# MMAThijssen/catfish

Hardware: NVIDIA B200
Metric: raw_signal_samples_per_sec_resnetrnn_infer (higher is better)
Workload: dtype f16+e5m2 (fp16 product + e5m2 correction product, fp32 accumulate)

## Files before the change

### catfish_b200/build.py

```python

import os
import subprocess
import sys

HERE = os.path.dirname(os.path.abspath(__file__))
CSRC = os.path.join(HERE, "csrc")
INCLUDE = os.path.join(HERE, "..", "include")
LIB = os.environ.get("CF_LIB_OUT") or os.path.join(HERE, "libcatfish_b200.so")
SOURCES = ["api.cu", "k1_normalize.cu", "k6_intervals.cu", "k7_chunks.cu", "k8_split.cu", "k9_validate.cu", "k11_sweep.cu", "simt_engine.cu", "tc_engine.cu"]
NVCC_FLAGS = (["-DCF_PRECISE_ACT"] if os.environ.get("CF_PRECISE_ACT") else []) + os.environ.get("CF_EXTRA_DEFS", "").split() + ["-gencode", "arch=compute_100a,code=sm_100a", "-lineinfo", "-O3", "-std=c++17",
              "--expt-relaxed-constexpr", "-Xcompiler", "-fPIC,-O2,-Wall", "-Xptxas", "-v"]


def _nvcc():
    for cand in (os.environ.get("NVCC"), "/usr/local/cuda/bin/nvcc", "nvcc"):
        if cand and (os.path.sep not in cand or os.path.exists(cand)):
            return cand
    return "nvcc"


def needs_build():
    if not os.path.exists(LIB):
        return True
    t = os.path.getmtime(LIB)
    deps = [os.path.join(CSRC, f) for f in os.listdir(CSRC)] + [os.path.join(INCLUDE, "catfish_b200.h")]
    return any(os.path.getmtime(d) > t for d in deps)


def build(force=False, verbose=False):
    if not force and not needs_build():
        return LIB
    objs = []
    logs = []
    os.makedirs(os.path.join(HERE, "build"), exist_ok=True)
    procs = []
    for src in SOURCES:
        obj = os.path.join(HERE, "build", os.environ.get("CF_OBJ_TAG", "") + src.replace(".cu", ".o"))
        cmd = [_nvcc()] + NVCC_FLAGS + ["-c", os.path.join(CSRC, src), "-o", obj]
        procs.append((src, subprocess.Popen(cmd, stdout=subprocess.PIPE, stderr=subprocess.STDOUT, text=True)))
        objs.append(obj)
    failed = False
    for src, p in procs:
        out, _ = p.communicate()
        logs.append("== %s\n%s" % (src, out))
        if p.returncode != 0:
            failed = True
    log = "\n".join(logs)
    with open(os.path.join(HERE, "build", "nvcc.log"), "w") as f:
        f.write(log)
    if failed:
        sys.stderr.write(log)
        raise RuntimeError("nvcc failed; see catfish_b200/build/nvcc.log")
    cmd = [_nvcc(), "-shared", "-o", LIB] + objs + ["-gencode", "arch=compute_100a,code=sm_100a"]
    r = subprocess.run(cmd, stdout=subprocess.PIPE, stderr=subprocess.STDOUT, text=True)
    if r.returncode != 0:
        sys.stderr.write(r.stdout)
        raise RuntimeError("link failed")
    if verbose:
        print(log)
    return LIB


if __name__ == "__main__":
    print(build(force="--force" in sys.argv, verbose="-v" in sys.argv))
```

### catfish_b200/csrc/tc_engine.cu

```cuda
#include <algorithm>
#include <cmath>
#include <cstdlib>
#include <cstring>
#include <type_traits>

#include "model.cuh"
#include "tc_ptx.cuh"

namespace cf {

using namespace ptx;

constexpr int kH = 64;
constexpr int kC = 32;
constexpr int kNX = 3 * kH;
constexpr int kTcChunkTiles = 2368;
constexpr float kGateScale = -1.4426950408889634f;
constexpr float kCandScale = 2.8853900817779268f;

constexpr int kFmtBf16x3 = 0, kFmtF16E5 = 1;

struct ConvParams {
    static constexpr int kFloats = 10 * 32;
    static constexpr int kW2 = kFloats * 4;
    static constexpr int kW3 = kW2 + 3 * 4096;
    static constexpr int kW45 = kW3 + 4096;
    static constexpr int kW6 = kW45 + 8192;
    static constexpr int kW7 = kW6 + 3 * 4096;
    static constexpr int kBytes = kW7 + 4096;
};

static void pack_b_operand(const float* w, int K, int N, int ldw, int col0, std::vector<__nv_bfloat16>* out,
                           float scale = 1.f, int n_split = 1 << 30, float scale_hi = 1.f) {
    const size_t plane = (size_t)K * N;
    const size_t base = out->size();
    out->resize(base + 2 * plane);
    __nv_bfloat16* hi = out->data() + base;
    __nv_bfloat16* lo = hi + plane;
    for (int k = 0; k < K; ++k)
        for (int n = 0; n < N; ++n) {
            const float v = w[(size_t)k * ldw + col0 + n] * (n < n_split ? scale : scale_hi);
            const __nv_bfloat16 h = __float2bfloat16_rn(v);
            const __nv_bfloat16 l = __float2bfloat16_rn(v - __bfloat162float(h));
            const size_t idx = ((size_t)(k / 8) * N + n) * 8 + (k % 8);
            hi[idx] = h;
            lo[idx] = l;
        }
}

static void pack_b_operand_f16e5(const float* w, int K, int N, int ldw, int col0, std::vector<__nv_bfloat16>* out,
                                 float scale = 1.f, int n_split = 1 << 30, float scale_hi = 1.f) {
    const size_t plane = (size_t)K * N;
    const size_t base = out->size();
    out->resize(base + 2 * plane);
    uint16_t* main = reinterpret_cast<uint16_t*>(out->data() + base);
    uint8_t* corr = reinterpret_cast<uint8_t*>(out->data() + base + plane);
    for (int k = 0; k < K; ++k)
        for (int n = 0; n < N; ++n) {
            const float v = w[(size_t)k * ldw + col0 + n] * (n < n_split ? scale : scale_hi);
            const __half h = __float2half_rn(v);
            const float hf = __half2float(h);
            const __half hs = __float2half_rn(hf * kCorrScale);
            main[((size_t)(k / 8) * N + n) * 8 + (k % 8)] = *reinterpret_cast<const uint16_t*>(&hs);
            const int c = k / 16, kc = k % 16;
            corr[((size_t)(2 * c) * N + n) * 16 + kc] = (uint8_t)__nv_cvt_float_to_fp8(hf / kCorrScale, __NV_SATFINITE, __NV_E5M2);
            corr[((size_t)(2 * c + 1) * N + n) * 16 + kc] = (uint8_t)__nv_cvt_float_to_fp8((v - hf) * kCorrScale, __NV_SATFINITE, __NV_E5M2);
        }
}

struct TcLayer {
    int in = 0;
    DevBuf wfused;
    int fmt = 0;
    DevBuf bz;
    DevBuf wxz;
};

struct TcEngine {
    SimtEnginePtr simt;
    DevBuf conv_params;
    int conv_nres = 0;
    std::vector<TcLayer> layers;
    DevBuf head_w;
    float head_b = 0.f;
    int n_sms = 148;
#ifdef CF_TRACE_PROBES
    bool trace_done = false;
    const char* trace_path = nullptr;
#endif
    int fmt = kFmtBf16x3;
};

bool tc_supported(const HostModel& hm) {
    if (hm.n_res() > 0 && hm.conv_channels() > kC) return false;
    if (hm.n_rnn() > 0 && hm.desc.layer_size > kH) return false;
    return true;
}

static HostModel pad_model(const HostModel& hm) {
    HostModel p = hm;
    if (hm.n_res() > 0) {
        const int C = hm.conv_channels();
        p.desc.layer_size_res = kC;
        for (size_t i = 0; i < hm.convs.size(); ++i) {
            const ConvLayer& s = hm.convs[i];
            ConvLayer& d = p.convs[i];
            const bool scalar_in = i < 2;
            d.cin = scalar_in ? 1 : kC;
            d.cout = kC;
            d.w.assign((size_t)d.k * d.cin * kC, 0.f);
            d.b.assign(kC, 0.f);
            for (int co = 0; co < C; ++co) d.b[co] = s.b[co];
            for (int k = 0; k < s.k; ++k)
                for (int ci = 0; ci < s.cin; ++ci)
                    for (int co = 0; co < C; ++co) d.w[((size_t)k * d.cin + ci) * kC + co] = s.w[((size_t)k * s.cin + ci) * C + co];
        }
    }
    auto unit2 = [](int r, int H) { return r < H ? r : kH + (r - H); };
    if (hm.n_rnn() > 0) {
        const int H = hm.desc.layer_size;
        p.desc.layer_size = kH;
        auto col = [&](int j) { return (j / H) * kH + j % H; };
        for (size_t i = 0; i < hm.gru.size(); ++i) {
            const GruDir& s = hm.gru[i];
            GruDir& d = p.gru[i];
            const bool first = i < 2;
            d.in = first ? (hm.n_res() > 0 ? kC : 1) : 2 * kH;
            d.h = kH;
            d.wx.assign((size_t)d.in * kNX, 0.f);
            d.bx.assign(kNX, 0.f);
            d.wgh.assign((size_t)kH * 2 * kH, 0.f);
            d.wch.assign((size_t)kH * kH, 0.f);
            for (int r = 0; r < s.in; ++r)
                for (int j = 0; j < 3 * H; ++j) d.wx[(size_t)(first ? r : unit2(r, H)) * kNX + col(j)] = s.wx[(size_t)r * 3 * H + j];
            for (int j = 0; j < 3 * H; ++j) d.bx[col(j)] = s.bx[j];
            for (int r = 0; r < H; ++r) {
                for (int j = 0; j < 2 * H; ++j) d.wgh[(size_t)r * 2 * kH + col(j)] = s.wgh[(size_t)r * 2 * H + j];
                for (int j = 0; j < H; ++j) d.wch[(size_t)r * kH + j] = s.wch[(size_t)r * H + j];
            }
        }
        p.head_w.assign(2 * kH, 0.f);
        for (int r = 0; r < 2 * H; ++r) p.head_w[unit2(r, H)] = hm.head_w[r];
    } else {
        p.head_w.assign(kC, 0.f);
        std::copy(hm.head_w.begin(), hm.head_w.end(), p.head_w.begin());
    }
    return p;
}

void EngineDelete::operator()(TcEngine* e) const { delete e; }

static int tc_set_attributes();

int tc_create(const HostModel& narrow, TcEnginePtr* out) {
    CF_TRY(tc_set_attributes());
    TcEnginePtr e(new TcEngine());
    int dev = 0;
    CF_CUDA(cudaGetDevice(&dev));
    CF_CUDA(cudaDeviceGetAttribute(&e->n_sms, cudaDevAttrMultiProcessorCount, dev));
    if (narrow.n_res() == 0) CF_TRY(simt_create(narrow, &e->simt));
    const HostModel hm = pad_model(narrow);
#ifdef CF_TRACE_PROBES
    e->trace_path = getenv("CF_TC_TRACE");
#endif
    {
        const bool covered = (hm.desc.network_type == CF_NET_RESNET_RNN && hm.n_res() == 2 && hm.conv_channels() == kC) ||
                             hm.desc.network_type == CF_NET_RNN;
        float wmax = 0.f;
        for (const GruDir& g : hm.gru) {
            for (float v : g.wx) wmax = std::max(wmax, std::fabs(v));
            for (float v : g.wgh) wmax = std::max(wmax, std::fabs(v));
            for (float v : g.wch) wmax = std::max(wmax, std::fabs(v));
        }
        const bool in_range = wmax * kCandScale * kCorrScale < 60000.f;
        e->fmt = covered && in_range ? kFmtF16E5 : kFmtBf16x3;
    }
    if (hm.n_res() >= 1) {
        const int n_extra = std::max(hm.n_res() - 2, 0);
        std::vector<uint8_t> all((size_t)(1 + n_extra) * ConvParams::kBytes, 0);
        uint8_t* blk = all.data();
        float* fp = reinterpret_cast<float*>(blk);
        auto put = [&](int slot, const std::vector<float>& v) { memcpy(fp + 32 * slot, v.data(), 32 * sizeof(float)); };
        auto put_w = [&](int off, const float* w, int n, int ldw, int col0, int dst_col0, int n_total) {
            __nv_bfloat16* hi = reinterpret_cast<__nv_bfloat16*>(blk + off);
            __nv_bfloat16* lo = hi + 32 * n_total;
            for (int k = 0; k < 32; ++k)
                for (int j = 0; j < n; ++j) {
                    const float v = w[(size_t)k * ldw + col0 + j];
                    const __nv_bfloat16 h = __float2bfloat16_rn(v);
                    const size_t idx = ((size_t)(k / 8) * n_total + dst_col0 + j) * 8 + (k % 8);
                    hi[idx] = h;
                    lo[idx] = __float2bfloat16_rn(v - __bfloat162float(h));
                }
        };
        auto put_block1 = [&](int i) {
            put(6, hm.convs[i].b); put(7, hm.convs[i + 1].b); put(8, hm.convs[i + 2].b); put(9, hm.convs[i + 3].b);
            put_w(ConvParams::kW45, hm.convs[i].w.data(), 32, 32, 0, 0, 64);
            put_w(ConvParams::kW45, hm.convs[i + 1].w.data(), 32, 32, 0, 32, 64);
            for (int tap = 0; tap < 3; ++tap) put_w(ConvParams::kW6 + tap * 4096, hm.convs[i + 2].w.data() + tap * 32 * 32, 32, 32, 0, 0, 32);
            put_w(ConvParams::kW7, hm.convs[i + 3].w.data(), 32, 32, 0, 0, 32);
        };
        put(0, hm.convs[0].w); put(1, hm.convs[0].b);
        put(2, hm.convs[1].w); put(3, hm.convs[1].b);
        put(4, hm.convs[2].b); put(5, hm.convs[3].b);
        for (int tap = 0; tap < 3; ++tap) put_w(ConvParams::kW2 + tap * 4096, hm.convs[2].w.data() + tap * 32 * 32, 32, 32, 0, 0, 32);
        put_w(ConvParams::kW3, hm.convs[3].w.data(), 32, 32, 0, 0, 32);
        if (hm.n_res() >= 2) put_block1(4);
        for (int b = 2; b < hm.n_res(); ++b) {
            blk = all.data() + (size_t)(b - 1) * ConvParams::kBytes;
            fp = reinterpret_cast<float*>(blk);
            put_block1(4 * b);
        }
        CF_TRY(e->conv_params.upload(all));
        e->conv_nres = hm.n_res();
    }
    e->layers.resize(hm.n_rnn());
    for (int l = 0; l < hm.n_rnn(); ++l) {
        TcLayer& L = e->layers[l];
        L.in = hm.gru[2 * l].in;
        L.fmt = L.in == kC ? kFmtBf16x3 : e->fmt;
        std::vector<__nv_bfloat16> wf;
        for (int d = 0; d < 2; ++d) {
            const GruDir& g = hm.gru[2 * l + d];
            auto pack = L.fmt == kFmtF16E5 ? pack_b_operand_f16e5 : pack_b_operand;
            if (L.in > 1) pack(g.wx.data(), L.in, kNX, kNX, 0, &wf, kGateScale, 2 * kH, kCandScale);
            pack(g.wgh.data(), kH, 2 * kH, 2 * kH, 0, &wf, kGateScale, 1 << 30, 1.f);
            pack(g.wch.data(), kH, kH, kH, 0, &wf, kCandScale, 1 << 30, 1.f);
        }
        CF_TRY(L.wfused.upload(wf));
        std::vector<float> bz(2 * kNX);
        for (int d = 0; d < 2; ++d)
            for (int j = 0; j < kNX; ++j)
                bz[d * kNX + j] = hm.gru[2 * l + d].bx[j] * (j < 2 * kH ? kGateScale : kCandScale);
        CF_TRY(L.bz.upload(bz));
        if (L.in == 1) {
            std::vector<float> wxz(2 * kNX);
            for (int d = 0; d < 2; ++d)
                for (int j = 0; j < kNX; ++j)
                    wxz[d * kNX + j] = hm.gru[2 * l + d].wx[j] * (j < 2 * kH ? kGateScale : kCandScale);
            CF_TRY(L.wxz.upload(wxz));
        }
    }
    CF_TRY(e->head_w.upload(hm.head_w));
    e->head_b = hm.head_b;
    *out = std::move(e);
    return CF_OK;
}

int tc_operand_format(const TcEngine* e) { return e ? e->fmt : 0; }
bool tc_can_emit_bits(const TcEngine* e) { return e && !e->layers.empty(); }

constexpr uint32_t kSliceBytes = 2u * 128 * kC * 2;
constexpr uint32_t kConvSmem = ConvParams::kBytes + 10 * kSliceBytes + 35 * 128 * 4 + 256;

__device__ __forceinline__ void store_a_row16(uint8_t* slice, int row, int c0, const float* v) {
#pragma unroll
    for (int g = 0; g < 2; ++g) {
        uint32_t hi[4], lo[4];
#pragma unroll
        for (int i = 0; i < 4; ++i) split_bf16x2(v[g * 8 + 2 * i], v[g * 8 + 2 * i + 1], hi[i], lo[i]);
        uint8_t* dst = slice + (c0 / 8 + g) * 2048 + row * 16;
        *reinterpret_cast<uint4*>(dst) = make_uint4(hi[0], hi[1], hi[2], hi[3]);
        *reinterpret_cast<uint4*>(dst + 8192) = make_uint4(lo[0], lo[1], lo[2], lo[3]);
    }
}

template <int N>
__device__ __forceinline__ void conv_mma_pred(uint32_t tmem_d, uint32_t a_slice, uint32_t w_mat, bool first, uint32_t elected) {
    constexpr uint32_t idesc = make_idesc_bf16(128, N);
#pragma unroll
    for (int pass = 0; pass < 3; ++pass) {
        const uint32_t ap = a_slice + (pass == 1 ? 8192u : 0u);
        const uint32_t wp = w_mat + (pass == 2 ? (uint32_t)(kC * N * 2) : 0u);
#pragma unroll
        for (int kk = 0; kk < 2; ++kk)
            umma_bf16_pred(tmem_d, make_smem_desc(ap + kk * 4096, 2048, 128), make_smem_desc(wp + kk * 2 * (N * 16), N * 16, 128),
                           idesc, !(first && pass == 0 && kk == 0), elected);
    }
}

__global__ void __launch_bounds__(288, 1)
tc_conv2_kernel(const uint8_t* __restrict__ params, const int16_t* __restrict__ raw, const double* __restrict__ stats,
                const float* __restrict__ xwin, const int64_t* __restrict__ src, const int32_t* __restrict__ valid,
                const int32_t* __restrict__ read, int64_t tile0, int n_tiles, __nv_bfloat16* __restrict__ y_out) {
    extern __shared__ __align__(128) uint8_t smem[];
    uint8_t* prm = smem;
    uint8_t* o1 = smem + ConvParams::kBytes;
    uint8_t* o2 = o1 + 4 * kSliceBytes;
    uint8_t* y0 = o2 + kSliceBytes;
    uint8_t* p1 = y0 + kSliceBytes;
    uint8_t* p2 = p1 + 3 * kSliceBytes;
    float* xs = reinterpret_cast<float*>(p2 + kSliceBytes);
    uint64_t* bars = reinterpret_cast<uint64_t*>(xs + 35 * 128);
    uint32_t* tmem_slot = reinterpret_cast<uint32_t*>(bars + 4);
    const float* fp = reinterpret_cast<const float*>(prm);
    uint64_t* bar_ready = &bars[0];
    uint64_t* bar_mma = &bars[1];
    uint64_t* bar_prm = &bars[2];

    const int warp = threadIdx.x >> 5, lane = threadIdx.x & 31;
    if (threadIdx.x == 0) {
        mbar_init(bar_ready, 8);
        mbar_init(bar_mma, 1);
        mbar_init(bar_prm, 1);
        fence_mbar_init();
        mbar_expect_tx(bar_prm, ConvParams::kBytes);
        bulk_g2s(prm, params, ConvParams::kBytes, bar_prm);
    }
    if (warp == 8) tmem_alloc<512>(tmem_slot);
    tc_fence_before_sync();
    __syncthreads();
    tc_fence_after_sync();
    const uint32_t tmem = *tmem_slot;
    constexpr int kLastU = kWindow + 1;
    mbar_wait(bar_prm, 0);

    if (warp == 8) {
        const uint32_t elected = elect_one();
        const uint32_t prm_u = smem_u32(prm);
        const uint32_t o1_u = smem_u32(o1), o2_u = smem_u32(o2);
        uint32_t it = 0;
        for (int tile = blockIdx.x; tile < n_tiles; tile += gridDim.x) {
            for (int u = 0; u <= kLastU; ++u, ++it) {
                mbar_wait(bar_ready, it & 1);
                tc_fence_after_sync();
                const int t1 = u - 1, t2 = u - 2;
                if (t1 >= 0 && t1 < kWindow) {
                    bool first = true;
#pragma unroll
                    for (int tap = 0; tap < 3; ++tap) {
                        const int tt = t1 + tap - 1;
                        if (tt < 0 || tt >= kWindow) continue;
                        conv_mma_pred<32>(tmem + 0, o1_u + (tt & 3) * kSliceBytes, prm_u + ConvParams::kW2 + tap * 4096, first, elected);
                        first = false;
                    }
                }
                if (t2 >= 0 && t2 < kWindow) conv_mma_pred<32>(tmem + 32, o2_u, prm_u + ConvParams::kW3, true, elected);
                umma_commit_pred(bar_mma, elected);
            }
        }
    } else {
        const int q = warp & 3, ch = warp >> 2;
        const int row = q * 32 + lane;
        const int c0 = ch * 16;
        const uint32_t t_lane = tmem + ((uint32_t)(q * 32) << 16) + c0;
        auto relu_bias = [&](uint32_t* r, int slot, float* v) {
#pragma unroll
            for (int i = 0; i < 16; i += 4) {
                const float4 b4 = *reinterpret_cast<const float4*>(fp + 32 * slot + c0 + i);
                v[i] = fmaxf(__uint_as_float(r[i]) + b4.x, 0.f);
                v[i + 1] = fmaxf(__uint_as_float(r[i + 1]) + b4.y, 0.f);
                v[i + 2] = fmaxf(__uint_as_float(r[i + 2]) + b4.z, 0.f);
                v[i + 3] = fmaxf(__uint_as_float(r[i + 3]) + b4.w, 0.f);
            }
        };
        auto make_o1 = [&](int t) {
            const float x = xs[t * 128 + row];
            float v[16];
#pragma unroll
            for (int i = 0; i < 16; ++i) v[i] = fmaxf(fmaf(x, fp[64 + c0 + i], fp[96 + c0 + i]), 0.f);
            store_a_row16(o1 + (t & 3) * kSliceBytes, row, c0, v);
        };
        uint32_t it = 0;
        for (int tile = blockIdx.x; tile < n_tiles; tile += gridDim.x) {
            asm volatile("bar.sync 1, 256;" ::: "memory");
            {
                const int64_t g = (tile0 + tile) * kTileWindows + row;
                const int nv = valid[g];
                const int64_t s0 = src[g];
                double shift = 0.0, scale = 1.0;
                if (raw && nv > 0) { const int r = read[g]; shift = stats[2 * r]; scale = stats[2 * r + 1]; }
                const int tb = ch ? 18 : 0, te = ch ? kWindow : 18;
                for (int t = tb; t < te; ++t) {
                    float v = 0.f;
                    if (t < nv) v = raw ? (float)(((double)raw[s0 + t] - shift) / scale) : xwin[s0 + t];
                    xs[t * 128 + row] = v;
                }
            }
            asm volatile("bar.sync 1, 256;" ::: "memory");
            make_o1(0);
            make_o1(1);
            fence_proxy_async_smem();
            tc_fence_before_sync();
            __syncwarp();
            if (lane == 0) mbar_arrive(bar_ready);
            for (int u = 0; u <= kLastU; ++u, ++it) {
                const int t1 = u - 1, t2 = u - 2;
                const bool h1 = t1 >= 0 && t1 < kWindow, h2 = t2 >= 0 && t2 < kWindow;
                mbar_wait(bar_mma, it & 1);
                tc_fence_after_sync();
                uint32_t r1[16], r2[16];
                if (h1) tmem_ld16_nowait(t_lane + 0, r1);
                if (h2) tmem_ld16_nowait(t_lane + 32, r2);
                tmem_ld_wait();
                tc_fence_before_sync();
                float v[16];
                if (h1) { relu_bias(r1, 4, v); store_a_row16(o2, row, c0, v); }
                if (h2) {
                    relu_bias(r2, 5, v);
                    const float x = xs[t2 * 128 + row];
#pragma unroll
                    for (int i = 0; i < 16; ++i) v[i] = fmaxf(v[i] + fmaf(x, fp[c0 + i], fp[32 + c0 + i]), 0.f);
                    store_a_row16(reinterpret_cast<uint8_t*>(y_out) + ((size_t)tile * kWindow + t2) * kSliceBytes, row, c0, v);
                }
                if (u < kLastU) {
                    fence_proxy_async_smem();
                    __syncwarp();
                    if (lane == 0) mbar_arrive(bar_ready);
                }
                if (u + 2 < kWindow) make_o1(u + 2);
            }
        }
    }
    tc_fence_before_sync();
    __syncthreads();
    if (warp == 8) tmem_dealloc<512>(tmem);
}


template <int FMT>
__device__ __forceinline__ void split4(float v0, float v1, float v2, float v3, int i, uint32_t* m8, uint32_t* s8) {
    if (FMT == kFmtBf16x3) {
        split_bf16x2(v0, v1, m8[i >> 1], s8[i >> 1]);
        split_bf16x2(v2, v3, m8[(i >> 1) + 1], s8[(i >> 1) + 1]);
    } else {
        uint32_t la, lb;
        split_f16e5x2(v0, v1, m8[i >> 1], la);
        split_f16e5x2(v2, v3, m8[(i >> 1) + 1], lb);
        s8[i >> 2] = la | (lb << 16);
        s8[4 + (i >> 2)] = f16e5_hi4(m8[i >> 1], m8[(i >> 1) + 1]);
    }
}

template <int FMT>
__device__ __forceinline__ void store_a_row16_f(uint8_t* slice, int row, int c0, const float* v) {
    uint32_t m8[8], s8[8];
#pragma unroll
    for (int i = 0; i < 16; i += 4) split4<FMT>(v[i], v[i + 1], v[i + 2], v[i + 3], i, m8, s8);
    uint8_t* dst = slice + (c0 / 8) * 2048 + row * 16;
    *reinterpret_cast<uint4*>(dst) = make_uint4(m8[0], m8[1], m8[2], m8[3]);
    *reinterpret_cast<uint4*>(dst + 2048) = make_uint4(m8[4], m8[5], m8[6], m8[7]);
    *reinterpret_cast<uint4*>(dst + 8192) = make_uint4(s8[0], s8[1], s8[2], s8[3]);
    *reinterpret_cast<uint4*>(dst + 8192 + 2048) = make_uint4(s8[4], s8[5], s8[6], s8[7]);
}
template <int FMT>
__device__ __forceinline__ void store_a_tmem16_f(uint32_t t_slot, const float* v) {
    uint32_t m8[8], s8[8];
#pragma unroll
    for (int i = 0; i < 16; i += 4) split4<FMT>(v[i], v[i + 1], v[i + 2], v[i + 3], i, m8, s8);
    tmem_st8_u32(t_slot, m8);
    tmem_st8_u32(t_slot + 16, s8);
}

constexpr uint32_t kConv4Smem = ConvParams::kBytes + 2 * kSliceBytes + 4 * (32 * 128 * 4) + 35 * 128 * 4 + 256;

template <int N>
__device__ __forceinline__ void conv_mma_ts_pred(uint32_t tmem_d, uint32_t tmem_a, uint32_t w_mat, bool first, uint32_t elected) {
    constexpr uint32_t idesc = make_idesc_bf16(128, N);
#pragma unroll
    for (int pass = 0; pass < 3; ++pass) {
        const uint32_t ap = tmem_a + (pass == 1 ? 16u : 0u);
        const uint32_t wp = w_mat + (pass == 2 ? (uint32_t)(kC * N * 2) : 0u);
#pragma unroll
        for (int kk = 0; kk < 2; ++kk)
            umma_bf16_ts_pred(tmem_d, ap + kk * 8, make_smem_desc(wp + kk * 2 * (N * 16), N * 16, 128), idesc,
                              !(first && pass == 0 && kk == 0), elected);
    }
}

__global__ void __launch_bounds__(576, 1)
tc_conv4_kernel(const uint8_t* __restrict__ params, const int16_t* __restrict__ raw, const double* __restrict__ stats,
                const float* __restrict__ xwin, const int64_t* __restrict__ src, const int32_t* __restrict__ valid,
                const int32_t* __restrict__ read, int64_t tile0, int n_tiles, __nv_bfloat16* __restrict__ y_out,
                const float* __restrict__ head_w, float* __restrict__ head_part) {
    constexpr int kFmt = kFmtBf16x3;
    extern __shared__ __align__(128) uint8_t smem[];
    uint8_t* prm = smem;
    uint8_t* o2 = smem + ConvParams::kBytes;
    uint8_t* p2 = o2 + kSliceBytes;
    float* sc_ring = reinterpret_cast<float*>(p2 + kSliceBytes);
    float* xs = sc_ring + 4 * 32 * 128;
    uint64_t* bars = reinterpret_cast<uint64_t*>(xs + 35 * 128);
    uint64_t* bar_ready_x = &bars[0];
    uint64_t* bar_mma_x = &bars[1];
    uint64_t* bar_ready_y = &bars[2];
    uint64_t* bar_mma_y = &bars[3];
    uint64_t* bar_prm = &bars[4];
    uint64_t* bar_y0_full = &bars[5];
    uint64_t* bar_y0_empty = &bars[8];
    uint32_t* tmem_slot = reinterpret_cast<uint32_t*>(bars + 11);
    const float* fp = reinterpret_cast<const float*>(prm);

    const int warp = threadIdx.x >> 5, lane = threadIdx.x & 31;
    if (threadIdx.x == 0) {
        mbar_init(bar_ready_x, 8);
        mbar_init(bar_mma_x, 1);
        mbar_init(bar_ready_y, 8);
        mbar_init(bar_mma_y, 1);
        mbar_init(bar_prm, 1);
        for (int i = 0; i < 3; ++i) { mbar_init(&bar_y0_full[i], 8); mbar_init(&bar_y0_empty[i], 1); }
        fence_mbar_init();
        mbar_expect_tx(bar_prm, ConvParams::kBytes);
        bulk_g2s(prm, params, ConvParams::kBytes, bar_prm);
    }
    if (warp == 16) tmem_alloc<512>(tmem_slot);
    tc_fence_before_sync();
    __syncthreads();
    tc_fence_after_sync();
    const uint32_t tmem = *tmem_slot;
    constexpr int kLastX = kWindow + 1;
    constexpr int kFirstY = 3, kLastY = kWindow + 5;
    constexpr uint32_t kTmScp1 = 128, kTmY0 = 192, kTmO1 = 288, kTmP1 = 416;
    mbar_wait(bar_prm, 0);

    if (warp == 16) {
        const uint32_t elected = elect_one();
        const uint32_t prm_u = smem_u32(prm), o2_u = smem_u32(o2);
        uint32_t it = 0;
        for (int tile = blockIdx.x; tile < n_tiles; tile += gridDim.x) {
            for (int u = 0; u <= kLastX; ++u, ++it) {
                mbar_wait(bar_ready_x, it & 1);
                tc_fence_after_sync();
                const int t1 = u - 1, t2 = u - 2;
                if (t1 >= 0 && t1 < kWindow) {
                    bool first = true;
#pragma unroll
                    for (int tap = 0; tap < 3; ++tap) {
                        const int tt = t1 + tap - 1;
                        if (tt < 0 || tt >= kWindow) continue;
                        conv_mma_ts_pred<32>(tmem + 0, tmem + kTmO1 + (tt & 3) * 32, prm_u + ConvParams::kW2 + tap * 4096, first, elected);
                        first = false;
                    }
                }
                if (t2 >= 0 && t2 < kWindow) conv_mma_pred<32>(tmem + 32, o2_u, prm_u + ConvParams::kW3, true, elected);
                umma_commit_pred(bar_mma_x, elected);
            }
        }
    } else if (warp == 17) {
        const uint32_t elected = elect_one();
        const uint32_t prm_u = smem_u32(prm), p2_u = smem_u32(p2);
        uint32_t it = 0, ny = 0, ny_slot = 0, ny_par = 0;
        for (int tile = blockIdx.x; tile < n_tiles; tile += gridDim.x) {
            for (int u = kFirstY; u <= kLastY; ++u, ++it) {
                mbar_wait(bar_ready_y, it & 1);
                tc_fence_after_sync();
                const int t3 = u - 3, t4 = u - 5, t5 = u - 6;
                if (t3 < kWindow) {
                    mbar_wait(&bar_y0_full[ny_slot], ny_par);
                    tc_fence_after_sync();
                    conv_mma_ts_pred<64>(tmem + kTmScp1, tmem + kTmY0 + ny_slot * 32, prm_u + ConvParams::kW45, true, elected);
                    umma_commit_pred(&bar_y0_empty[ny_slot], elected);
                    ++ny;
                    if (++ny_slot == 3) { ny_slot = 0; ny_par ^= 1; }
                }
                if (t4 >= 0 && t4 < kWindow) {
                    bool first = true;
#pragma unroll
                    for (int tap = 0; tap < 3; ++tap) {
                        const int tt = t4 + tap - 1;
                        if (tt < 0 || tt >= kWindow) continue;
                        conv_mma_ts_pred<32>(tmem + 64, tmem + kTmP1 + (tt % 3) * 32, prm_u + ConvParams::kW6 + tap * 4096, first, elected);
                        first = false;
                    }
                }
                if (t5 >= 0 && t5 < kWindow) conv_mma_pred<32>(tmem + 96, p2_u, prm_u + ConvParams::kW7, true, elected);
                umma_commit_pred(bar_mma_y, elected);
            }
        }
    } else {
        const int ew = warp & 7;
        const int q = ew & 3, ch = ew >> 2;
        const int row = q * 32 + lane;
        const int c0 = ch * 16;
        const uint32_t t_row = tmem + ((uint32_t)(q * 32) << 16);
        const uint32_t t_lane = t_row + c0;
        const uint32_t t_opnd = t_row + ch * 8;
        auto relu_bias = [&](uint32_t* r, int slot, float* v) {
#pragma unroll
            for (int i = 0; i < 16; i += 4) {
                const float4 b4 = *reinterpret_cast<const float4*>(fp + 32 * slot + c0 + i);
                const float2 s0 = fadd2(make_float2(__uint_as_float(r[i]), __uint_as_float(r[i + 1])), make_float2(b4.x, b4.y));
                const float2 s1 = fadd2(make_float2(__uint_as_float(r[i + 2]), __uint_as_float(r[i + 3])), make_float2(b4.z, b4.w));
                v[i] = fmaxf(s0.x, 0.f);
                v[i + 1] = fmaxf(s0.y, 0.f);
                v[i + 2] = fmaxf(s1.x, 0.f);
                v[i + 3] = fmaxf(s1.y, 0.f);
            }
        };
        if (warp < 8) {
            auto make_o1 = [&](int t) {
                const float2 x = splat2(xs[t * 128 + row]);
                float v[16];
#pragma unroll
                for (int i = 0; i < 16; i += 2) {
                    const float2 o = ffma2(x, *reinterpret_cast<const float2*>(fp + 64 + c0 + i), *reinterpret_cast<const float2*>(fp + 96 + c0 + i));
                    v[i] = fmaxf(o.x, 0.f);
                    v[i + 1] = fmaxf(o.y, 0.f);
                }
                store_a_tmem16_f<kFmt>(t_opnd + kTmO1 + (t & 3) * 32, v);
            };
            uint32_t it = 0, ny = 0, ny_slot = 0, ny_par = 1;
            for (int tile = blockIdx.x; tile < n_tiles; tile += gridDim.x) {
                asm volatile("bar.sync 1, 256;" ::: "memory");
                {
                    const int64_t g = (tile0 + tile) * kTileWindows + row;
                    const int nv = valid[g];
                    const int64_t s0 = src[g];
                    double shift = 0.0, scale = 1.0;
                    if (raw && nv > 0) { const int r = read[g]; shift = stats[2 * r]; scale = stats[2 * r + 1]; }
                    const int tb = ch ? 18 : 0, te = ch ? kWindow : 18;
                    for (int t = tb; t < te; ++t) {
                        float v = 0.f;
                        if (t < nv) v = raw ? (float)(((double)raw[s0 + t] - shift) / scale) : xwin[s0 + t];
                        xs[t * 128 + row] = v;
                    }
                }
                asm volatile("bar.sync 1, 256;" ::: "memory");
                make_o1(0);
                make_o1(1);
                tmem_st_wait();
                tc_fence_before_sync();
                __syncwarp();
                if (lane == 0) mbar_arrive(bar_ready_x);
                for (int u = 0; u <= kLastX; ++u, ++it) {
                    const int t1 = u - 1, t2 = u - 2;
                    const bool h1 = t1 >= 0 && t1 < kWindow, h2 = t2 >= 0 && t2 < kWindow;
                    mbar_wait(bar_mma_x, it & 1);
                    tc_fence_after_sync();
                    uint32_t r1[16], r2[16];
                    if (h1) tmem_ld16_nowait(t_lane + 0, r1);
                    if (h2) tmem_ld16_nowait(t_lane + 32, r2);
                    tmem_ld_wait();
                    float v[16];
                    if (h1) { relu_bias(r1, 4, v); store_a_row16_f<kFmt>(o2, row, c0, v); }
                    if (u < kLastX) {
                        fence_proxy_async_smem();
                        tmem_st_wait();
                        tc_fence_before_sync();
                        __syncwarp();
                        if (lane == 0) mbar_arrive(bar_ready_x);
                    }
                    if (h2) {
                        relu_bias(r2, 5, v);
                        const float2 x = splat2(xs[t2 * 128 + row]);
#pragma unroll
                        for (int i = 0; i < 16; i += 2) {
                            const float2 sc = ffma2(x, *reinterpret_cast<const float2*>(fp + c0 + i), *reinterpret_cast<const float2*>(fp + 32 + c0 + i));
                            const float2 o = fadd2(make_float2(v[i], v[i + 1]), sc);
                            v[i] = fmaxf(o.x, 0.f);
                            v[i + 1] = fmaxf(o.y, 0.f);
                        }
                        if (ny >= 3) mbar_wait(&bar_y0_empty[ny_slot], ny_par);
                        tc_fence_after_sync();
                        store_a_tmem16_f<kFmt>(t_opnd + kTmY0 + ny_slot * 32, v);
                        tmem_st_wait();
                        tc_fence_before_sync();
                        __syncwarp();
                        if (lane == 0) mbar_arrive(&bar_y0_full[ny_slot]);
                        ++ny;
                        if (++ny_slot == 3) { ny_slot = 0; ny_par ^= 1; }
                    }
                    if (u + 2 < kWindow) make_o1(u + 2);
                }
            }
        } else {
            float* sc_mine = sc_ring + c0 * 128 + row;
            uint32_t it = 0;
            if (lane == 0) mbar_arrive(bar_ready_y);
            for (int tile = blockIdx.x; tile < n_tiles; tile += gridDim.x) {
                for (int u = kFirstY; u <= kLastY; ++u, ++it) {
                    const int t3 = u - 3, t4 = u - 5, t5 = u - 6;
                    const bool h3 = t3 < kWindow, h4 = t4 >= 0 && t4 < kWindow, h5 = t5 >= 0 && t5 < kWindow;
                    mbar_wait(bar_mma_y, it & 1);
                    tc_fence_after_sync();
                    uint32_t r3[16], r4[16], r5[16], rs[16];
                    if (h3) {
                        tmem_ld16_nowait(t_lane + kTmScp1 + 32, r3);
                        tmem_ld16_nowait(t_lane + kTmScp1, rs);
                    }
                    if (h4) tmem_ld16_nowait(t_lane + 64, r4);
                    if (h5) tmem_ld16_nowait(t_lane + 96, r5);
                    tmem_ld_wait();
                    float v[16];
                    if (h3) { relu_bias(r3, 7, v); store_a_tmem16_f<kFmt>(t_opnd + kTmP1 + (t3 % 3) * 32, v); }
                    if (h4) { relu_bias(r4, 8, v); store_a_row16_f<kFmt>(p2, row, c0, v); }
                    fence_proxy_async_smem();
                    tmem_st_wait();
                    tc_fence_before_sync();
                    __syncwarp();
                    if (lane == 0) mbar_arrive(bar_ready_y);
                    if (h3) {
                        float* dst = sc_mine + (t3 & 3) * 4096;
#pragma unroll
                        for (int i = 0; i < 16; ++i) dst[i * 128] = __uint_as_float(rs[i]) + fp[192 + c0 + i];
                    }
                    if (h5) {
                        relu_bias(r5, 9, v);
                        const float* sc = sc_mine + (t5 & 3) * 4096;
#pragma unroll
                        for (int i = 0; i < 16; i += 2) {
                            const float2 o = fadd2(make_float2(v[i], v[i + 1]), make_float2(sc[i * 128], sc[(i + 1) * 128]));
                            v[i] = fmaxf(o.x, 0.f);
                            v[i + 1] = fmaxf(o.y, 0.f);
                        }
                        if (head_w) {
                            float2 acc2 = make_float2(0.f, 0.f);
#pragma unroll
                            for (int i = 0; i < 16; i += 2)
                                acc2 = ffma2(make_float2(v[i], v[i + 1]), __ldg(reinterpret_cast<const float2*>(head_w + c0 + i)), acc2);
                            head_part[(((size_t)tile * kWindow + t5) * 2 + ch) * 128 + row] = acc2.x + acc2.y;
                        } else {
                            store_a_row16_f<kFmt>(reinterpret_cast<uint8_t*>(y_out) + ((size_t)tile * kWindow + t5) * kSliceBytes, row, c0, v);
                        }
                    }
                }
            }
        }
    }
    tc_fence_before_sync();
    __syncthreads();
    if (warp == 16) tmem_dealloc<512>(tmem);
}

constexpr int kBlockRing = 4;
constexpr uint32_t kBlockSmem = ConvParams::kBytes + (kBlockRing + 3 + 1) * kSliceBytes + 256;

__global__ void __launch_bounds__(320, 1)
tc_conv_block_kernel(const uint8_t* __restrict__ params, const __nv_bfloat16* __restrict__ y_in, int n_tiles,
                     __nv_bfloat16* __restrict__ y_out) {
    constexpr int kFmt = kFmtBf16x3;
    extern __shared__ __align__(128) uint8_t smem[];
    uint8_t* prm = smem;
    uint8_t* yin = smem + ConvParams::kBytes;
    uint8_t* p1 = yin + kBlockRing * kSliceBytes;
    uint8_t* p2 = p1 + 3 * kSliceBytes;
    uint64_t* bars = reinterpret_cast<uint64_t*>(p2 + kSliceBytes);
    uint64_t* bar_ready = &bars[0];
    uint64_t* bar_mma = &bars[1];
    uint64_t* bar_prm = &bars[2];
    uint64_t* bar_full = &bars[3];
    uint64_t* bar_empty = &bars[3 + kBlockRing];
    uint32_t* tmem_slot = reinterpret_cast<uint32_t*>(bars + 3 + 2 * kBlockRing);
    const float* fp = reinterpret_cast<const float*>(prm);

    const int warp = threadIdx.x >> 5, lane = threadIdx.x & 31;
    if (threadIdx.x == 0) {
        mbar_init(bar_ready, 8);
        mbar_init(bar_mma, 1);
        mbar_init(bar_prm, 1);
        for (int i = 0; i < kBlockRing; ++i) { mbar_init(&bar_full[i], 1); mbar_init(&bar_empty[i], 1); }
        fence_mbar_init();
        mbar_expect_tx(bar_prm, ConvParams::kBytes);
        bulk_g2s(prm, params, ConvParams::kBytes, bar_prm);
    }
    if (warp == 8) tmem_alloc<512>(tmem_slot);
    tc_fence_before_sync();
    __syncthreads();
    tc_fence_after_sync();
    const uint32_t tmem = *tmem_slot;
    constexpr int kLastU = kWindow + 2;
    constexpr uint32_t kTmP2 = 256, kTmP3 = 288;
    mbar_wait(bar_prm, 0);

    if (warp == 8) {
        const uint32_t elected = elect_one();
        const uint32_t prm_u = smem_u32(prm), yin_u = smem_u32(yin), p1_u = smem_u32(p1), p2_u = smem_u32(p2);
        uint32_t it = 0, n = 0;
        for (int tile = blockIdx.x; tile < n_tiles; tile += gridDim.x) {
            for (int u = 0; u <= kLastU; ++u, ++it) {
                mbar_wait(bar_ready, it & 1);
                tc_fence_after_sync();
                const int t2 = u - 2, t3 = u - 3;
                if (u < kWindow) {
                    const uint32_t slot = n % kBlockRing;
                    mbar_wait(&bar_full[slot], (n / kBlockRing) & 1);
                    conv_mma_pred<64>(tmem + (u & 3) * 64, yin_u + slot * kSliceBytes, prm_u + ConvParams::kW45, true, elected);
                    umma_commit_pred(&bar_empty[slot], elected);
                    ++n;
                }
                if (t2 >= 0 && t2 < kWindow) {
                    bool first = true;
#pragma unroll
                    for (int tap = 0; tap < 3; ++tap) {
                        const int tt = t2 + tap - 1;
                        if (tt < 0 || tt >= kWindow) continue;
                        conv_mma_pred<32>(tmem + kTmP2, p1_u + (tt % 3) * kSliceBytes, prm_u + ConvParams::kW6 + tap * 4096, first, elected);
                        first = false;
                    }
                }
                if (t3 >= 0 && t3 < kWindow) conv_mma_pred<32>(tmem + kTmP3, p2_u, prm_u + ConvParams::kW7, true, elected);
                umma_commit_pred(bar_mma, elected);
            }
        }
    } else if (warp == 9) {
        if (lane == 0) {
            const uint8_t* src = reinterpret_cast<const uint8_t*>(y_in);
            uint32_t n = 0;
            for (int tile = blockIdx.x; tile < n_tiles; tile += gridDim.x)
                for (int t = 0; t < kWindow; ++t, ++n) {
                    const uint32_t slot = n % kBlockRing;
                    if (n >= kBlockRing) mbar_wait(&bar_empty[slot], (n / kBlockRing - 1) & 1);
                    mbar_expect_tx(&bar_full[slot], kSliceBytes);
                    bulk_g2s(yin + slot * kSliceBytes, src + ((size_t)tile * kWindow + t) * kSliceBytes, kSliceBytes, &bar_full[slot]);
                }
        }
    } else {
        const int q = warp & 3, ch = warp >> 2;
        const int row = q * 32 + lane;
        const int c0 = ch * 16;
        const uint32_t t_lane = tmem + ((uint32_t)(q * 32) << 16) + c0;
        auto relu_bias = [&](uint32_t* r, int slot, float* v) {
#pragma unroll
            for (int i = 0; i < 16; i += 4) {
                const float4 b4 = *reinterpret_cast<const float4*>(fp + 32 * slot + c0 + i);
                const float2 s0 = fadd2(make_float2(__uint_as_float(r[i]), __uint_as_float(r[i + 1])), make_float2(b4.x, b4.y));
                const float2 s1 = fadd2(make_float2(__uint_as_float(r[i + 2]), __uint_as_float(r[i + 3])), make_float2(b4.z, b4.w));
                v[i] = fmaxf(s0.x, 0.f);
                v[i + 1] = fmaxf(s0.y, 0.f);
                v[i + 2] = fmaxf(s1.x, 0.f);
                v[i + 3] = fmaxf(s1.y, 0.f);
            }
        };
        uint32_t it = 0;
        if (lane == 0) mbar_arrive(bar_ready);
        for (int tile = blockIdx.x; tile < n_tiles; tile += gridDim.x) {
            for (int u = 0; u <= kLastU; ++u, ++it) {
                const int t2 = u - 2, t3 = u - 3;
                const bool h1 = u < kWindow, h2 = t2 >= 0 && t2 < kWindow, h3 = t3 >= 0 && t3 < kWindow;
                mbar_wait(bar_mma, it & 1);
                tc_fence_after_sync();
                uint32_t r1[16], r2[16], r3[16], rs[16];
                if (h1) tmem_ld16_nowait(t_lane + (u & 3) * 64 + 32, r1);
                if (h2) tmem_ld16_nowait(t_lane + kTmP2, r2);
                if (h3) {
                    tmem_ld16_nowait(t_lane + kTmP3, r3);
                    tmem_ld16_nowait(t_lane + (t3 & 3) * 64, rs);
                }
                tmem_ld_wait();
                float v[16];
                if (h1) { relu_bias(r1, 7, v); store_a_row16_f<kFmt>(p1 + (u % 3) * kSliceBytes, row, c0, v); }
                if (h2) { relu_bias(r2, 8, v); store_a_row16_f<kFmt>(p2, row, c0, v); }
                fence_proxy_async_smem();
                tc_fence_before_sync();
                __syncwarp();
                if (lane == 0) mbar_arrive(bar_ready);
                if (h3) {
                    relu_bias(r3, 9, v);
#pragma unroll
                    for (int i = 0; i < 16; i += 2) {
                        const float2 sc = fadd2(make_float2(__uint_as_float(rs[i]), __uint_as_float(rs[i + 1])),
                                                *reinterpret_cast<const float2*>(fp + 192 + c0 + i));
                        const float2 o = fadd2(make_float2(v[i], v[i + 1]), sc);
                        v[i] = fmaxf(o.x, 0.f);
                        v[i + 1] = fmaxf(o.y, 0.f);
                    }
                    store_a_row16_f<kFmt>(reinterpret_cast<uint8_t*>(y_out) + ((size_t)tile * kWindow + t3) * kSliceBytes, row, c0, v);
                }
            }
        }
    }
    tc_fence_before_sync();
    __syncthreads();
    if (warp == 8) tmem_dealloc<512>(tmem);
}

template <int KX> struct GruF2Cfg {
    static constexpr bool kNoX = KX == 1;
    static constexpr int kChunks = KX / 16;
    static constexpr int kStages = KX == 128 ? 8 : 10;
    static constexpr uint32_t kWx = 0;
    static constexpr uint32_t kWgh = kWx + (kNoX ? 0u : 2u * KX * kNX * 2);
    static constexpr uint32_t kWch = kWgh + 2u * kH * 128 * 2;
    static constexpr uint32_t kWBytes = kWch + 2u * kH * 64 * 2;
    static constexpr uint32_t kRing = kWBytes;
    static constexpr uint32_t kBias = kRing + (uint32_t)kStages * 8192;
    static constexpr uint32_t kBars = kBias + 2 * 192 * 4;
    static constexpr uint32_t kSmem = kBars + 512;
    static constexpr int kBarG = 0, kBarC = 1, kBarRh = 2, kBarH = 3, kBarCfree = 4, kBarXdone = 5;
    static constexpr int kBarFull = 16, kBarEmpty = 16 + kStages, kBarTma = 16 + 2 * kStages, kBarW = 16 + 3 * kStages;
};
__host__ __device__ constexpr uint32_t gru_out_block_bytes(int fmt) { return fmt == kFmtF16E5 ? 49152u : 65536u; }
constexpr int kGruF2Threads = 768;
constexpr int kGruF2Converters = 2;
constexpr int kGruF2EpiRegs = 96, kGruF2ServiceRegs = 48;

template <int KX, int FMT, int FMT_OUT>
__global__ void __launch_bounds__(kGruF2Threads, 1)
tc_gru_fused2_kernel(const uint8_t* __restrict__ wpk, const float* __restrict__ bias,
                     const __nv_bfloat16* __restrict__ x_blocks, __nv_bfloat16* __restrict__ y_out,
                     const float* __restrict__ head_w, float* __restrict__ head_part, int n_tiles,
                     long long* __restrict__ trace, const float* __restrict__ x_scalar, const float* __restrict__ wx_scalar) {
    using Cfg = GruF2Cfg<KX>;
    constexpr bool kNoX = Cfg::kNoX;
#ifdef CF_TRACE_PROBES
    int tr_n = 0;
#define CF_TR(region, step, tag)                                                                   \
    do {                                                                                           \
        if (trace && blockIdx.x == 0 && (step) >= 36 && (step) < 40 && tr_n < 200) {               \
            trace[((region) * 200 + tr_n) * 2] = (tag) + 1000 * (long long)(step);                      \
            trace[((region) * 200 + tr_n) * 2 + 1] = clock64();                                    \
            ++tr_n;                                                                                \
        }                                                                                          \
    } while (0)
#else
#define CF_TR(region, step, tag) do { } while (0)
#endif
#ifdef CF_TRACE_CHUNKS
#define CF_TRC(region, step, tag) CF_TR(region, step, tag)
#else
#define CF_TRC(region, step, tag) do { } while (0)
#endif
    extern __shared__ __align__(128) uint8_t smem[];
    uint64_t* bars = reinterpret_cast<uint64_t*>(smem + Cfg::kBars);
    uint64_t* w_bar = &bars[Cfg::kBarW];
    uint32_t* tmem_slot = reinterpret_cast<uint32_t*>(&bars[Cfg::kBarW + 1]);
    float* bias_s = reinterpret_cast<float*>(smem + Cfg::kBias);

    const int warp = threadIdx.x >> 5, lane = threadIdx.x & 31;
    const int dir = blockIdx.x & 1;
    const int slot = blockIdx.x >> 1, n_slots = gridDim.x >> 1;
    const int stride = 2 * n_slots;
    auto tiles_of = [&](int chain) -> int {
        const int first = slot * 2 + chain;
        return first < n_tiles ? (n_tiles - first + stride - 1) / stride : 0;
    };
    auto blk_of = [&](int chain, int gs) -> size_t {
        const int ti = gs / kWindow, s = gs - ti * kWindow;
        return (size_t)(slot * 2 + chain + ti * stride) * kWindow + (dir ? kWindow - 1 - s : s);
    };

    if (threadIdx.x == 0) {
        for (int c = 0; c < 2; ++c) {
            uint64_t* b = &bars[8 * c];
            mbar_init(&b[Cfg::kBarG], 1);
            mbar_init(&b[Cfg::kBarC], 1);
            mbar_init(&b[Cfg::kBarRh], 16);
            mbar_init(&b[Cfg::kBarH], 16);
            mbar_init(&b[Cfg::kBarCfree], 16);
            mbar_init(&b[Cfg::kBarXdone], 1);
        }
        for (int i = 0; i < Cfg::kStages; ++i) {
            mbar_init(&bars[Cfg::kBarFull + i], 1);
            mbar_init(&bars[Cfg::kBarEmpty + i], 1);
            mbar_init(&bars[Cfg::kBarTma + i], 1);
        }
        mbar_init(w_bar, 1);
        fence_mbar_init();
    }
#ifndef CF_PRECISE_ACT
    if (threadIdx.x < 192) bias_s[threadIdx.x] = bias[dir * kNX + threadIdx.x] * (threadIdx.x < 2 * kH ? kSigArgScale : kTanhArgScale);
    if (kNoX && threadIdx.x < 192) bias_s[192 + threadIdx.x] = wx_scalar[dir * kNX + threadIdx.x] * (threadIdx.x < 2 * kH ? kSigArgScale : kTanhArgScale);
#else
    if (threadIdx.x < 192) bias_s[threadIdx.x] = bias[dir * kNX + threadIdx.x];
    if (kNoX && threadIdx.x < 192) bias_s[192 + threadIdx.x] = wx_scalar[dir * kNX + threadIdx.x];
#endif
    if (warp == 16) tmem_alloc<512>(tmem_slot);
    tc_fence_before_sync();
    __syncthreads();
    tc_fence_after_sync();
    const uint32_t tmem = *tmem_slot;

    if (warp >= 16) {
    asm volatile("setmaxnreg.dec.sync.aligned.u32 %0;" ::"n"(kGruF2ServiceRegs));
    if (warp == 18) {
        if (lane == 0) {
            mbar_expect_tx(w_bar, Cfg::kWBytes);
            const uint8_t* wsrc = wpk + (size_t)dir * Cfg::kWBytes;
            for (uint32_t off = 0; off < Cfg::kWBytes; off += 32768) {
                const uint32_t n = Cfg::kWBytes - off < 32768 ? Cfg::kWBytes - off : 32768;
                bulk_g2s(smem + off, wsrc + off, n, w_bar);
            }
            constexpr bool kCompact = FMT == kFmtF16E5;
            constexpr size_t plane = (size_t)128 * KX * 2;
            constexpr size_t blk_bytes = kCompact ? plane + (size_t)(KX / 16) * 2048 : 2 * plane;
            const uint8_t* xbase = reinterpret_cast<const uint8_t*>(x_blocks);
            const int total0 = tiles_of(0) * kWindow, total1 = tiles_of(1) * kWindow;
            uint32_t st = 0, par = 1;
            for (int gs = 0; gs < (kNoX ? 0 : total0); ++gs) {
                for (int c = 0; c < 2; ++c) {
                    if (c == 1 && gs >= total1) break;
                    const uint8_t* xb = xbase + blk_of(c, gs) * blk_bytes;
                    if (kCompact) {
                        const int nc = (c == 0 && gs < total1) ? 1 : 0, ngs = nc ? gs : gs + 1;
                        if (ngs < total0 && (nc == 0 || ngs < total1)) {
                            const uint8_t* nb = xbase + blk_of(nc, ngs) * blk_bytes;
                            bulk_prefetch_l2(nb, (uint32_t)plane);
                            bulk_prefetch_l2(nb + plane, (uint32_t)(KX / 16) * 2048);
                        }
                    }
                    for (int kk = 0; kk < Cfg::kChunks; ++kk) {
                        mbar_wait(&bars[Cfg::kBarEmpty + st], par);
                        CF_TRC(5, gs, 80 + kk);
                        uint8_t* dst = smem + Cfg::kRing + st * 8192;
                        uint64_t* landed = &bars[(kCompact ? Cfg::kBarTma : Cfg::kBarFull) + st];
                        if (kCompact) {
                            mbar_expect_tx(landed, 6144);
                            bulk_g2s(dst, xb + kk * 4096, 4096, landed);
                            bulk_g2s(dst + 4096, xb + plane + kk * 2048, 2048, landed);
                        } else {
                            mbar_expect_tx(landed, 8192);
                            bulk_g2s(dst, xb + kk * 4096, 4096, landed);
                            bulk_g2s(dst + 4096, xb + plane + kk * 4096, 4096, landed);
                        }
                        if (++st == Cfg::kStages) { st = 0; par ^= 1; }
                    }
                }
            }
        }
    } else if (warp >= 19) {
        if (FMT == kFmtF16E5 && warp < 19 + kGruF2Converters) {
            static_assert(Cfg::kStages % kGruF2Converters == 0, "converter warps split the ring by stage");
            const int total0 = tiles_of(0) * kWindow, total1 = tiles_of(1) * kWindow;
            const int n_chunks = (total0 + total1) * Cfg::kChunks;
            uint32_t st = warp - 19, par = 0;
            for (int cn = warp - 19; cn < n_chunks; cn += kGruF2Converters) {
                mbar_wait(&bars[Cfg::kBarTma + st], par);
                if (lane == 0 && warp == 19) CF_TRC(4, cn / (2 * Cfg::kChunks), 70);
                uint8_t* stage = smem + Cfg::kRing + st * 8192;
#pragma unroll
                for (int r = 0; r < 4; ++r) {
                    const int row = r * 32 + lane;
                    const uint4 a = *reinterpret_cast<const uint4*>(stage + row * 16);
                    const uint4 b = *reinterpret_cast<const uint4*>(stage + 2048 + row * 16);
                    *reinterpret_cast<uint4*>(stage + 6144 + row * 16) =
                        make_uint4(f16e5_hi4(a.x, a.y), f16e5_hi4(a.z, a.w), f16e5_hi4(b.x, b.y), f16e5_hi4(b.z, b.w));
                }
                fence_proxy_async_smem();
                __syncwarp();
                if (lane == 0) mbar_arrive(&bars[Cfg::kBarFull + st]);
                if (lane == 0 && warp == 19) CF_TRC(4, cn / (2 * Cfg::kChunks), 71);
                if ((st += kGruF2Converters) >= Cfg::kStages) { st -= Cfg::kStages; par ^= 1; }
            }
        }
    } else if (warp >= 16 && warp < 18) {
        {
            constexpr bool kE5 = FMT == kFmtF16E5;
            constexpr uint32_t idesc_g = kE5 ? make_idesc_f16(128, 2 * kH) : make_idesc_bf16(128, 2 * kH);
            constexpr uint32_t idesc_c = kE5 ? make_idesc_f16(128, kH) : make_idesc_bf16(128, kH);
            constexpr uint32_t idesc_x = kE5 ? make_idesc_f16(128, kNX) : make_idesc_bf16(128, kNX);
            constexpr uint32_t idesc_g8 = make_idesc_e5m2(128, 2 * kH), idesc_c8 = make_idesc_e5m2(128, kH);
            constexpr uint32_t idesc_x8 = make_idesc_e5m2(128, kNX);
            const uint32_t elected = elect_one();
            const int c = warp - 16;
            const uint32_t s0 = smem_u32(smem);
            uint64_t* b = &bars[8 * c];
            const uint32_t dg = tmem + c * 256, dc = dg + 2 * kH, ta = dg + 3 * kH;
            const int total = tiles_of(c) * kWindow;
            const int total1 = tiles_of(1) * kWindow;
            mbar_wait(w_bar, 0);
            for (int gs = 0; gs < total; ++gs) {
                const uint32_t par = gs & 1;
                uint32_t cn = (uint32_t)(c == 0 ? gs + (gs < total1 ? gs : total1) : 2 * gs + 1) * Cfg::kChunks;
                if (kNoX) {
                } else if (c == 1) mbar_wait(&bars[Cfg::kBarXdone], gs & 1);
                else if (gs > 0 && gs - 1 < total1) mbar_wait(&bars[8 + Cfg::kBarXdone], (gs - 1) & 1);
                if (gs > 0) mbar_wait(&b[Cfg::kBarCfree], (gs - 1) & 1);
                if (lane == 0) CF_TR(c, gs, 10);
                auto issue_x = [&](auto st0c) {
                    constexpr int kSt0 = decltype(st0c)::value;
                    static_assert(kSt0 + Cfg::kChunks <= Cfg::kStages || kNoX, "an entry does not wrap around the ring");
                    uint32_t ring_lo = (uint32_t)make_smem_desc(s0 + Cfg::kRing, 2048, 128);
                    uint32_t wx_lo = (uint32_t)make_smem_desc(s0 + Cfg::kWx, kNX * 16, 128);
                    asm volatile("" : "+r"(ring_lo), "+r"(wx_lo));
                    constexpr uint64_t ahi = make_smem_desc(0, 2048, 128) & 0xffffffff00000000ull;
                    constexpr uint64_t bhi = make_smem_desc(0, kNX * 16, 128) & 0xffffffff00000000ull;
                    const uint32_t xpar = (cn / Cfg::kStages) & 1;
#pragma unroll
                    for (int kk = 0; kk < Cfg::kChunks; ++kk) {
                        const int st = kSt0 + kk;
                        mbar_wait(&bars[Cfg::kBarFull + st], xpar);
                        if (lane == 0) CF_TRC(c, gs, 60 + kk);
                        tc_fence_after_sync();
                        const uint32_t a_lo = ring_lo + st * (8192 >> 4), w_lo = wx_lo + kk * (2 * kNX * 16 >> 4);
                        if (kE5) {
                            umma_bf16_pred(dg, ahi | a_lo, bhi | w_lo, idesc_x, kk != 0, elected);
                            umma_f8_pred(dg, ahi | (a_lo + (4096 >> 4)), bhi | (w_lo + (KX * kNX * 2 >> 4)), idesc_x8, 1, elected);
                        } else {
#pragma unroll
                            for (int pass = 0; pass < 3; ++pass)
                                umma_bf16_pred(dg, ahi | (a_lo + (pass == 1 ? 4096 >> 4 : 0)),
                                               bhi | (w_lo + (pass == 2 ? KX * kNX * 2 >> 4 : 0)), idesc_x, (kk | pass) != 0, elected);
                        }
                        umma_commit_pred(&bars[Cfg::kBarEmpty + st], elected);
                        if (lane == 0) CF_TRC(c, gs, 20 + kk);
                        if (kk == Cfg::kChunks - 1 && lane == 0) CF_TR(c, gs, 27);
                    }
                };
                if constexpr (kNoX) {
                } else if constexpr (Cfg::kChunks == Cfg::kStages) {
                    issue_x(std::integral_constant<int, 0>{});
                } else {
                    static_assert(Cfg::kStages == 10 && Cfg::kChunks == 2, "entries start at the even stages 0..8");
                    switch (cn % Cfg::kStages) {
                        case 0: issue_x(std::integral_constant<int, 0>{}); break;
                        case 2: issue_x(std::integral_constant<int, 2>{}); break;
                        case 4: issue_x(std::integral_constant<int, 4>{}); break;
                        case 6: issue_x(std::integral_constant<int, 6>{}); break;
                        default: issue_x(std::integral_constant<int, 8>{}); break;
                    }
                }
                if (!kNoX && lane == 0) mbar_arrive(&b[Cfg::kBarXdone]);
                uint32_t wgh_lo = (uint32_t)make_smem_desc(s0 + Cfg::kWgh, 128 * 16, 128);
                uint32_t wch_lo = (uint32_t)make_smem_desc(s0 + Cfg::kWch, 64 * 16, 128);
                asm volatile("" : "+r"(wgh_lo), "+r"(wch_lo));
                constexpr uint64_t ghi = make_smem_desc(0, 128 * 16, 128) & 0xffffffff00000000ull;
                constexpr uint64_t chi = make_smem_desc(0, 64 * 16, 128) & 0xffffffff00000000ull;
                mbar_wait(&b[Cfg::kBarH], par);
                if (lane == 0) CF_TR(c, gs, 30);
                tc_fence_after_sync();
                if (kE5) {
#pragma unroll
                    for (int kk = 0; kk < kH / 16; ++kk) {
                        const uint32_t w_lo = wgh_lo + kk * (2 * 128 * 16 >> 4);
                        umma_bf16_ts_pred(dg, ta + kk * 8, ghi | w_lo, idesc_g, !kNoX || kk != 0, elected);
                        umma_f8_ts_pred(dg, ta + 32 + kk * 8, ghi | (w_lo + (kH * 128 * 2 >> 4)), idesc_g8, 1, elected);
                    }
                } else {
#pragma unroll
                    for (int pass = 0; pass < 3; ++pass) {
                        const uint32_t ap = ta + (pass == 1 ? 32u : 0u);
#pragma unroll
                        for (int kk = 0; kk < kH / 16; ++kk)
                            umma_bf16_ts_pred(dg, ap + kk * 8, ghi | (wgh_lo + (pass == 2 ? kH * 128 * 2 >> 4 : 0) + kk * (2 * 128 * 16 >> 4)),
                                              idesc_g, !kNoX || (pass | kk) != 0, elected);
                    }
                }
                umma_commit_pred(&b[Cfg::kBarG], elected);
                if (lane == 0) CF_TR(c, gs, 31);
                mbar_wait(&b[Cfg::kBarRh], par);
                if (lane == 0) CF_TR(c, gs, 40);
                tc_fence_after_sync();
                if (kE5) {
#pragma unroll
                    for (int kk = 0; kk < kH / 16; ++kk) {
                        const uint32_t w_lo = wch_lo + kk * (2 * 64 * 16 >> 4);
                        umma_bf16_ts_pred(dc, ta + kk * 8, chi | w_lo, idesc_c, !kNoX || kk != 0, elected);
                        umma_f8_ts_pred(dc, ta + 32 + kk * 8, chi | (w_lo + (kH * 64 * 2 >> 4)), idesc_c8, 1, elected);
                    }
                } else {
#pragma unroll
                    for (int pass = 0; pass < 3; ++pass) {
                        const uint32_t ap = ta + (pass == 1 ? 32u : 0u);
#pragma unroll
                        for (int kk = 0; kk < kH / 16; ++kk)
                            umma_bf16_ts_pred(dc, ap + kk * 8, chi | (wch_lo + (pass == 2 ? kH * 64 * 2 >> 4 : 0) + kk * (2 * 64 * 16 >> 4)),
                                              idesc_c, !kNoX || (pass | kk) != 0, elected);
                    }
                }
                umma_commit_pred(&b[Cfg::kBarC], elected);
                if (lane == 0) CF_TR(c, gs, 41);
            }
        }
    }
    } else {
        asm volatile("setmaxnreg.inc.sync.aligned.u32 %0;" ::"n"(kGruF2EpiRegs));
        const int q = warp & 3, us = warp >> 2;
        const int row = q * 32 + lane;
        const int j0 = us * 16;
        const uint32_t t_row = tmem + ((uint32_t)(q * 32) << 16);
        const int tot[2] = {tiles_of(0) * kWindow, tiles_of(1) * kWindow};
        float2 h2[2][8];
        int spos[2] = {0, 0};
        const uint32_t blk_step = dir ? 0xffffffffu : 1u;
        const uint32_t blk_jump = (uint32_t)stride * kWindow - blk_step * (kWindow - 1);
        uint32_t cblk[2] = {(uint32_t)(slot * 2) * kWindow + (dir ? kWindow - 1 : 0),
                            (uint32_t)(slot * 2 + 1) * kWindow + (dir ? kWindow - 1 : 0)};
        uint8_t* const y_main = reinterpret_cast<uint8_t*>(y_out) + ((size_t)(dir * kH + j0) / 8 * 128 + row) * 16;
        const int32_t y_lo_delta = FMT_OUT == kFmtF16E5
            ? 128 * 2 * kH * 2 + ((dir * kH + j0) / 16 * 128 + row) * 16 - ((dir * kH + j0) / 8 * 128 + row) * 16
            : 128 * 2 * kH * 2;
        float* const head_base = head_part + (dir * 4 + us) * 128 + row;
        const float* const xs_base = x_scalar + row;
#pragma unroll
        for (int c = 0; c < 2; ++c)
#pragma unroll
            for (int j = 0; j < 8; ++j) h2[c][j] = make_float2(0.f, 0.f);

        auto bias4 = [&](int idx, float xv) -> float4 {
            float4 b4 = *reinterpret_cast<const float4*>(bias_s + idx);
            if (kNoX) {
                const float4 w4 = *reinterpret_cast<const float4*>(bias_s + 192 + idx);
                b4.x = fmaf(xv, w4.x, b4.x); b4.y = fmaf(xv, w4.y, b4.y); b4.z = fmaf(xv, w4.z, b4.z); b4.w = fmaf(xv, w4.w, b4.w);
            }
            return b4;
        };
        auto sig4 = [&](const uint32_t* a, float4 b4, float2& o0, float2& o1) {
#ifndef CF_PRECISE_ACT
            o0 = sigmoid_zb2(make_float2(__uint_as_float(a[0]), __uint_as_float(a[1])), make_float2(b4.x, b4.y));
            o1 = sigmoid_zb2(make_float2(__uint_as_float(a[2]), __uint_as_float(a[3])), make_float2(b4.z, b4.w));
#else
            float z[4] = {__uint_as_float(a[0]) + b4.x, __uint_as_float(a[1]) + b4.y, __uint_as_float(a[2]) + b4.z, __uint_as_float(a[3]) + b4.w};
            float y[4];
            sigmoid4_z(z, y);
            o0 = make_float2(y[0], y[1]);
            o1 = make_float2(y[2], y[3]);
#endif
        };
        auto tanh4v = [&](const uint32_t* a, float4 b4, float2& o0, float2& o1) {
#ifndef CF_PRECISE_ACT
            o0 = tanh_zb2(make_float2(__uint_as_float(a[0]), __uint_as_float(a[1])), make_float2(b4.x, b4.y));
            o1 = tanh_zb2(make_float2(__uint_as_float(a[2]), __uint_as_float(a[3])), make_float2(b4.z, b4.w));
#else
            float z[4] = {__uint_as_float(a[0]) + b4.x, __uint_as_float(a[1]) + b4.y, __uint_as_float(a[2]) + b4.z, __uint_as_float(a[3]) + b4.w};
            float y[4];
            tanh4_z(z, y);
            o0 = make_float2(y[0], y[1]);
            o1 = make_float2(y[2], y[3]);
#endif
        };
        auto begin_tile = [&](int c) {
            const uint32_t t_ahi = t_row + c * 256 + 3 * kH + j0 / 2, t_alo = t_ahi + 32;
            const uint32_t z[8] = {0, 0, 0, 0, 0, 0, 0, 0};
#pragma unroll
            for (int j = 0; j < 8; ++j) h2[c][j] = make_float2(0.f, 0.f);
            tmem_st8_u32(t_ahi, z);
            tmem_st8_u32(t_alo, z);
            tmem_st_wait();
            tc_fence_before_sync();
            __syncwarp();
            if (lane == 0) mbar_arrive(&bars[8 * c + Cfg::kBarH]);
        };
        auto phase_r = [&](int c, int gs) {
            uint64_t* b = &bars[8 * c];
            const uint32_t t_acc = t_row + c * 256 + j0;
            const uint32_t t_ahi = t_row + c * 256 + 3 * kH + j0 / 2, t_alo = t_ahi + 32;
            const float xv = kNoX ? __ldg(xs_base + (size_t)cblk[c] * 128) : 0.f;
            if (warp == 0 && lane == 0) CF_TR(2 + c, gs, 49);
            mbar_wait(&b[Cfg::kBarG], gs & 1);
            if (warp == 0 && lane == 0) CF_TR(2 + c, gs, 50);
            tc_fence_after_sync();
            uint32_t ar[16];
            tmem_ld16_nowait(t_acc, ar);
            tmem_ld_wait();
            uint32_t hi[8], lo[8];
#pragma unroll
            for (int i = 0; i < 16; i += 4) {
                float2 r0, r1;
                sig4(ar + i, bias4(j0 + i, xv), r0, r1);
                const float2 p0 = fmul2(r0, h2[c][i >> 1]), p1 = fmul2(r1, h2[c][(i >> 1) + 1]);
                split4<FMT>(p0.x, p0.y, p1.x, p1.y, i, hi, lo);
            }
            tmem_st8_u32(t_ahi, hi);
            tmem_st8_u32(t_alo, lo);
            tmem_st_wait();
            tc_fence_before_sync();
            __syncwarp();
            if (lane == 0) mbar_arrive(&b[Cfg::kBarRh]);
            if (warp == 0 && lane == 0) CF_TR(2 + c, gs, 51);
        };
        auto phase_c = [&](int c, int gs) {
            uint64_t* b = &bars[8 * c];
            const uint32_t t_acc = t_row + c * 256 + j0;
            const uint32_t t_ahi = t_row + c * 256 + 3 * kH + j0 / 2, t_alo = t_ahi + 32;
            const uint32_t blk = cblk[c];
            const int s = spos[c];
            const float xv = kNoX ? __ldg(xs_base + (size_t)blk * 128) : 0.f;
            float2 u2[8];
            {
                uint32_t au[16];
                tmem_ld16_nowait(t_acc + kH, au);
                tmem_ld_wait();
#pragma unroll
                for (int i = 0; i < 16; i += 4) sig4(au + i, bias4(kH + j0 + i, xv), u2[i >> 1], u2[(i >> 1) + 1]);
            }
            if (warp == 0 && lane == 0) CF_TR(2 + c, gs, 52);
            mbar_wait(&b[Cfg::kBarC], gs & 1);
            if (warp == 0 && lane == 0) CF_TR(2 + c, gs, 53);
            tc_fence_after_sync();
            uint32_t ac[16];
            tmem_ld16_nowait(t_acc + 2 * kH, ac);
            tmem_ld_wait();
            tc_fence_before_sync();
            __syncwarp();
            if (lane == 0) mbar_arrive(&b[Cfg::kBarCfree]);
            uint32_t hi[8], lo[8];
#pragma unroll
            for (int i = 0; i < 16; i += 4) {
                float2 c0v, c1v;
                tanh4v(ac + i, bias4(2 * kH + j0 + i, xv), c0v, c1v);
                float2& ha = h2[c][i >> 1];
                float2& hb = h2[c][(i >> 1) + 1];
                ha = ffma2(u2[i >> 1], ffma2(c0v, splat2(-1.f), ha), c0v);
                hb = ffma2(u2[(i >> 1) + 1], ffma2(c1v, splat2(-1.f), hb), c1v);
                split4<FMT>(ha.x, ha.y, hb.x, hb.y, i, hi, lo);
            }
            const bool more = gs + 1 < tot[c];
            if (s + 1 < kWindow) {
                tmem_st8_u32(t_ahi, hi);
                tmem_st8_u32(t_alo, lo);
                tmem_st_wait();
                tc_fence_before_sync();
                __syncwarp();
                if (lane == 0) mbar_arrive(&b[Cfg::kBarH]);
            }
            if (warp == 0 && lane == 0) CF_TR(2 + c, gs, 55);
            if (y_out) {
                if (FMT_OUT != FMT) {
#pragma unroll
                    for (int i = 0; i < 16; i += 4)
                        split4<FMT_OUT>(h2[c][i >> 1].x, h2[c][i >> 1].y, h2[c][(i >> 1) + 1].x, h2[c][(i >> 1) + 1].y, i, hi, lo);
                }
                uint8_t* ym = y_main + (size_t)blk * gru_out_block_bytes(FMT_OUT);
                *reinterpret_cast<uint4*>(ym) = make_uint4(hi[0], hi[1], hi[2], hi[3]);
                *reinterpret_cast<uint4*>(ym + 2048) = make_uint4(hi[4], hi[5], hi[6], hi[7]);
                *reinterpret_cast<uint4*>(ym + y_lo_delta) = make_uint4(lo[0], lo[1], lo[2], lo[3]);
                if (FMT_OUT != kFmtF16E5)
                    *reinterpret_cast<uint4*>(ym + y_lo_delta + 2048) = make_uint4(lo[4], lo[5], lo[6], lo[7]);
            }
            if (head_part) {
                const float* hw = head_w + dir * kH + j0;
                float2 acc2 = make_float2(0.f, 0.f);
#pragma unroll
                for (int i = 0; i < 8; ++i) acc2 = ffma2(h2[c][i], __ldg(reinterpret_cast<const float2*>(hw) + i), acc2);
                head_base[(size_t)blk * 1024] = acc2.x + acc2.y;
            }
            if (s + 1 == kWindow) {
                spos[c] = 0;
                cblk[c] = blk + blk_jump;
                if (more) begin_tile(c);
            } else {
                spos[c] = s + 1;
                cblk[c] = blk + blk_step;
            }
            if (warp == 0 && lane == 0) CF_TR(2 + c, gs, 56);
        };

        if (tot[0] > 0) begin_tile(0);
        if (tot[1] > 0) begin_tile(1);
        const int g_end = tot[0] > tot[1] ? tot[0] : tot[1];
        for (int g = 0; g <= g_end; ++g) {
            if (g < tot[0]) phase_r(0, g);
            if (g >= 1 && g - 1 < tot[1]) phase_c(1, g - 1);
            if (g < tot[0]) phase_c(0, g);
            if (g < tot[1]) phase_r(1, g);
        }
    }
    tc_fence_before_sync();
    __syncthreads();
    if (warp == 16) tmem_dealloc<512>(tmem);
}

#undef CF_TR
#undef CF_TRC

__global__ void __launch_bounds__(256)
tc_head_kernel(const float* __restrict__ head_part, int n_parts, float b, const int64_t* __restrict__ src,
               const int32_t* __restrict__ valid, const int32_t* __restrict__ read,
               const double* __restrict__ stats, int64_t tile0, int64_t n_rows, float* __restrict__ probs, int want_logits,
               unsigned* __restrict__ lwords, double threshold) {
    __shared__ float logit[kWindow][kTileWindows + 1];
    const int64_t tile = blockIdx.x;
    if (tile * kTileWindows * kWindow >= n_rows) return;
    for (int i = threadIdx.x; i < kWindow * kTileWindows; i += blockDim.x) {
        const int t = i / kTileWindows, w = i % kTileWindows;
        const size_t blk = (size_t)tile * kWindow + t;
        float acc = b;
        for (int k = 0; k < n_parts; ++k) acc += head_part[(blk * n_parts + k) * 128 + w];
        logit[t][w] = acc;
    }
    __syncthreads();
    for (int i = threadIdx.x; i < kWindow * kTileWindows; i += blockDim.x) {
        const int w = i / kWindow, t = i % kWindow;
        const int64_t g = (tile0 + tile) * kTileWindows + w;
        const bool real = t < valid[g];
        float p = 0.f;
        if (real) {
            p = want_logits ? logit[t][w] : 1.f / (1.f + expf(-logit[t][w]));
            if (stats) {
                const double sc = stats[2 * read[g] + 1];
                if (!(sc > 0.0)) p = nanf("");
            }
        }
        if (!lwords) {
            if (real) probs[src[g] + t] = p;
            continue;
        }
        const bool hit = real && (double)p >= threshold;
        const unsigned hits = __ballot_sync(0xffffffffu, hit);
        if (hit) {
            const int64_t sidx = src[g] + t;
            const unsigned peers = __match_any_sync(hits, (unsigned long long)(sidx >> 5));
            const unsigned bits = __reduce_or_sync(peers, 1u << (sidx & 31));
            if ((threadIdx.x & 31) == __ffs(peers) - 1) atomicOr(&lwords[sidx >> 5], bits);
        }
    }
}

__global__ void __launch_bounds__(256)
tc_head_conv_kernel(const __nv_bfloat16* __restrict__ y, const float* __restrict__ w, float b,
                    const int64_t* __restrict__ src, const int32_t* __restrict__ valid,
                    const int32_t* __restrict__ read, const double* __restrict__ stats,
                    int64_t tile0, int64_t n_rows, float* __restrict__ probs, int want_logits) {
    __shared__ float logit[kWindow][kTileWindows + 1];
    __shared__ float ws[kC];
    const int64_t tile = blockIdx.x;
    if (tile * kTileWindows * kWindow >= n_rows) return;
    if (threadIdx.x < kC) ws[threadIdx.x] = w[threadIdx.x];
    __syncthreads();
    for (int i = threadIdx.x; i < kWindow * kTileWindows; i += blockDim.x) {
        const int t = i / kTileWindows, wr = i % kTileWindows;
        const __nv_bfloat16* blk = y + ((size_t)tile * kWindow + t) * (2 * 128 * kC);
        float acc = b;
#pragma unroll
        for (int kg = 0; kg < kC / 8; ++kg) {
            const uint4 hi = *reinterpret_cast<const uint4*>(blk + ((size_t)kg * 128 + wr) * 8);
            const uint4 lo = *reinterpret_cast<const uint4*>(blk + 128 * kC + ((size_t)kg * 128 + wr) * 8);
            const uint32_t hw[4] = {hi.x, hi.y, hi.z, hi.w}, lw[4] = {lo.x, lo.y, lo.z, lo.w};
#pragma unroll
            for (int k = 0; k < 4; ++k) {
                const float v0 = __uint_as_float(hw[k] << 16) + __uint_as_float(lw[k] << 16);
                const float v1 = __uint_as_float(hw[k] & 0xffff0000u) + __uint_as_float(lw[k] & 0xffff0000u);
                acc = fmaf(v0, ws[kg * 8 + 2 * k], acc);
                acc = fmaf(v1, ws[kg * 8 + 2 * k + 1], acc);
            }
        }
        logit[t][wr] = acc;
    }
    __syncthreads();
    for (int i = threadIdx.x; i < kWindow * kTileWindows; i += blockDim.x) {
        const int wr = i / kWindow, t = i % kWindow;
        const int64_t g = (tile0 + tile) * kTileWindows + wr;
        if (t >= valid[g]) continue;
        float p = want_logits ? logit[t][wr] : 1.f / (1.f + expf(-logit[t][wr]));
        if (stats) {
            const double sc = stats[2 * read[g] + 1];
            if (!(sc > 0.0)) p = nanf("");
        }
        probs[src[g] + t] = p;
    }
}

int simt_conv_stack(SimtEngine* e, DevBuf* ws, const HostModel& hm, const int16_t* raw, const double* stats,
                    const float* xwin, WindowTable tab, int64_t tile0, int64_t tiles, int64_t chunk_tiles,
                    const float** feat, cudaStream_t stream, Profiler* prof);

static size_t tc_workspace_bytes(int64_t tiles) {
    const size_t blocks = (size_t)tiles * kWindow;
    size_t b = 0;
    b += blocks * 128 * kC * 2 * 2;
    b += 2 * blocks * 128 * 2 * kH * 2 * 2;
    b += blocks * 8 * 128 * 4;
    return b + 4096;
}

int tc_reserve(const TcEngine* e, DevBuf* ws, DevBuf* simt_ws, const HostModel& hm, int64_t n_tiles) {
    if (n_tiles <= 0) return CF_OK;
    const int64_t chunk = n_tiles < kTcChunkTiles ? n_tiles : kTcChunkTiles;
    CF_TRY(ws->ensure(tc_workspace_bytes(chunk)));
    if (!e->conv_params.ptr) CF_TRY(simt_conv_stack_reserve(simt_ws, hm, chunk));
    return CF_OK;
}

constexpr uint32_t kSmemPerSm = 228 * 1024;
static_assert(GruF2Cfg<128>::kSmem > kSmemPerSm / 2, "two tc_gru_fused2_kernel<128> CTAs could share an SM's TMEM");
static_assert(GruF2Cfg<32>::kSmem > kSmemPerSm / 2, "two tc_gru_fused2_kernel<32> CTAs could share an SM's TMEM");
static_assert(GruF2Cfg<1>::kSmem > kSmemPerSm / 2, "two tc_gru_fused2_kernel<1> CTAs could share an SM's TMEM");
static_assert(kConv4Smem > kSmemPerSm / 2, "two tc_conv4_kernel CTAs could share an SM's TMEM");
static_assert(kBlockSmem > kSmemPerSm / 2, "two tc_conv_block_kernel CTAs could share an SM's TMEM");
static_assert(kConvSmem > kSmemPerSm / 2, "two tc_conv2_kernel CTAs could share an SM's TMEM");

static int tc_set_attributes() {
    CF_CUDA(cudaFuncSetAttribute(tc_gru_fused2_kernel<1, 0, 0>, cudaFuncAttributeMaxDynamicSharedMemorySize, GruF2Cfg<1>::kSmem));
    CF_CUDA(cudaFuncSetAttribute(tc_gru_fused2_kernel<1, 1, 1>, cudaFuncAttributeMaxDynamicSharedMemorySize, GruF2Cfg<1>::kSmem));
    CF_CUDA(cudaFuncSetAttribute(tc_gru_fused2_kernel<32, 0, 0>, cudaFuncAttributeMaxDynamicSharedMemorySize, GruF2Cfg<32>::kSmem));
    CF_CUDA(cudaFuncSetAttribute(tc_gru_fused2_kernel<32, 0, 1>, cudaFuncAttributeMaxDynamicSharedMemorySize, GruF2Cfg<32>::kSmem));
    CF_CUDA(cudaFuncSetAttribute(tc_gru_fused2_kernel<128, 0, 0>, cudaFuncAttributeMaxDynamicSharedMemorySize, GruF2Cfg<128>::kSmem));
    CF_CUDA(cudaFuncSetAttribute(tc_gru_fused2_kernel<128, 1, 1>, cudaFuncAttributeMaxDynamicSharedMemorySize, GruF2Cfg<128>::kSmem));
    CF_CUDA(cudaFuncSetAttribute(tc_conv2_kernel, cudaFuncAttributeMaxDynamicSharedMemorySize, kConvSmem));
    CF_CUDA(cudaFuncSetAttribute(tc_conv4_kernel, cudaFuncAttributeMaxDynamicSharedMemorySize, kConv4Smem));
    CF_CUDA(cudaFuncSetAttribute(tc_conv_block_kernel, cudaFuncAttributeMaxDynamicSharedMemorySize, kBlockSmem));
    return CF_OK;
}

int tc_forward(TcEngine* e, DevBuf* ws, DevBuf* simt_ws, const HostModel& hm, const int16_t* raw, const double* stats,
               const float* xwin, WindowTable tab, int64_t n_tiles, float* probs, cudaStream_t stream, Profiler* prof,
               bool want_logits, const LabelBits* bits) {
    if (n_tiles <= 0) return CF_OK;
    if (bits && (e->layers.empty() || want_logits)) { set_error("label-bit output needs a GRU head"); return CF_ERR_BAD_ARG; }
    const int64_t chunk = n_tiles < kTcChunkTiles ? n_tiles : kTcChunkTiles;
    CF_TRY(ws->ensure(tc_workspace_bytes(chunk)));
    const size_t blocks_max = (size_t)chunk * kWindow;
    uint8_t* p = static_cast<uint8_t*>(ws->ptr);
    __nv_bfloat16* a0 = reinterpret_cast<__nv_bfloat16*>(p);
    p += blocks_max * 128 * kC * 2 * 2;
    __nv_bfloat16* ybuf[2];
    ybuf[0] = reinterpret_cast<__nv_bfloat16*>(p);
    p += blocks_max * 128 * 2 * kH * 2 * 2;
    ybuf[1] = reinterpret_cast<__nv_bfloat16*>(p);
    p += blocks_max * 128 * 2 * kH * 2 * 2;
    float* head_part = reinterpret_cast<float*>(p);

    const int n_layers = (int)e->layers.size();
    for (int64_t tile0 = 0; tile0 < n_tiles; tile0 += kTcChunkTiles) {
        const int64_t tiles = std::min<int64_t>(kTcChunkTiles, n_tiles - tile0);
        const int64_t blocks = tiles * kWindow;
        const int64_t rows = blocks * 128;
        const float* feat = nullptr;
        const __nv_bfloat16* a_in = nullptr;
        if (e->conv_params.ptr) {
            ProfScope ps(prof, KC_K2_CONV, stream);
            const int grid = (int)std::min<int64_t>(tiles, e->n_sms);
            const bool fused_head = n_layers == 0 && e->conv_nres == 2;
            if (e->conv_nres >= 2)
                tc_conv4_kernel<<<grid, 576, kConv4Smem, stream>>>(e->conv_params.as<uint8_t>(), raw, stats, xwin, tab.src,
                                                                  tab.valid, tab.read, tile0, (int)tiles, a0,
                                                                  fused_head ? e->head_w.as<float>() : nullptr,
                                                                  fused_head ? head_part : nullptr);
            else
                tc_conv2_kernel<<<grid, 288, kConvSmem, stream>>>(e->conv_params.as<uint8_t>(), raw, stats, xwin, tab.src, tab.valid,
                                                                  tab.read, tile0, (int)tiles, a0);
            CF_LAUNCHED();
            a_in = a0;
            for (int b = 2; b < e->conv_nres; ++b) {
                __nv_bfloat16* out = a_in == a0 ? ybuf[1] : a0;
                tc_conv_block_kernel<<<grid, 320, kBlockSmem, stream>>>(
                    e->conv_params.as<uint8_t>() + (size_t)(b - 1) * ConvParams::kBytes, a_in, (int)tiles, out);
                CF_LAUNCHED();
                a_in = out;
            }
        } else {
            CF_TRY(simt_conv_stack(e->simt.get(), simt_ws, hm, raw, stats, xwin, tab, tile0, tiles, chunk, &feat, stream, prof));
        }
        for (int l = 0; l < n_layers; ++l) {
            const TcLayer& L = e->layers[l];
            const bool last = l + 1 == n_layers;
            __nv_bfloat16* yo = last ? nullptr : ybuf[l & 1];
            ProfScope ps(prof, KC_K4_GRU, stream);
            long long* trace_dev = nullptr;
#ifdef CF_TRACE_PROBES
            if (e->trace_path && !e->trace_done && L.in != kC) {
                CF_CUDA(cudaMalloc(&trace_dev, 6 * 200 * 2 * sizeof(long long)));
                CF_CUDA(cudaMemsetAsync(trace_dev, 0, 6 * 200 * 2 * sizeof(long long), stream));
            }
#endif
            const int grid2 = 2 * (int)std::min<int64_t>((tiles + 1) / 2, e->n_sms / 2);
            const float* hw_l = last ? e->head_w.as<float>() : nullptr;
            float* hp_l = last ? head_part : nullptr;
            const int fmt_out = last ? L.fmt : e->layers[l + 1].fmt;
            if (L.in == 1) {
                if (L.fmt == kFmtF16E5)
                    tc_gru_fused2_kernel<1, 1, 1><<<grid2, kGruF2Threads, GruF2Cfg<1>::kSmem, stream>>>(
                        L.wfused.as<uint8_t>(), L.bz.as<float>(), nullptr, yo, hw_l, hp_l, (int)tiles, nullptr, feat, L.wxz.as<float>());
                else
                    tc_gru_fused2_kernel<1, 0, 0><<<grid2, kGruF2Threads, GruF2Cfg<1>::kSmem, stream>>>(
                        L.wfused.as<uint8_t>(), L.bz.as<float>(), nullptr, yo, hw_l, hp_l, (int)tiles, nullptr, feat, L.wxz.as<float>());
            } else if (L.in == kC) {
                if (fmt_out == kFmtF16E5)
                    tc_gru_fused2_kernel<32, 0, 1><<<grid2, kGruF2Threads, GruF2Cfg<32>::kSmem, stream>>>(
                        L.wfused.as<uint8_t>(), L.bz.as<float>(), a_in, yo, hw_l, hp_l, (int)tiles, nullptr, nullptr, nullptr);
                else
                    tc_gru_fused2_kernel<32, 0, 0><<<grid2, kGruF2Threads, GruF2Cfg<32>::kSmem, stream>>>(
                        L.wfused.as<uint8_t>(), L.bz.as<float>(), a_in, yo, hw_l, hp_l, (int)tiles, nullptr, nullptr, nullptr);
            } else if (L.fmt == kFmtF16E5) {
                tc_gru_fused2_kernel<128, 1, 1><<<grid2, kGruF2Threads, GruF2Cfg<128>::kSmem, stream>>>(
                    L.wfused.as<uint8_t>(), L.bz.as<float>(), a_in, yo, hw_l, hp_l, (int)tiles, trace_dev, nullptr, nullptr);
            } else {
                tc_gru_fused2_kernel<128, 0, 0><<<grid2, kGruF2Threads, GruF2Cfg<128>::kSmem, stream>>>(
                    L.wfused.as<uint8_t>(), L.bz.as<float>(), a_in, yo, hw_l, hp_l, (int)tiles, trace_dev, nullptr, nullptr);
            }
            CF_LAUNCHED();
#ifdef CF_TRACE_PROBES
            if (trace_dev) {
                CF_CUDA(cudaStreamSynchronize(stream));
                std::vector<long long> host(6 * 200 * 2);
                CF_CUDA(cudaMemcpy(host.data(), trace_dev, host.size() * sizeof(long long), cudaMemcpyDeviceToHost));
                if (FILE* f = fopen(e->trace_path, "w")) {
                    for (int rg = 0; rg < 6; ++rg)
                        for (int k = 0; k < 200; ++k)
                            if (host[(rg * 200 + k) * 2 + 1])
                                fprintf(f, "%d %lld %lld\n", rg, host[(rg * 200 + k) * 2], host[(rg * 200 + k) * 2 + 1]);
                    fclose(f);
                }
                cudaFree(trace_dev);
                e->trace_done = true;
            }
#endif
            a_in = yo;
        }
        if (n_layers == 0 && e->conv_nres == 2) {
            ProfScope ps(prof, KC_K5_HEAD, stream);
            tc_head_kernel<<<(unsigned)tiles, 256, 0, stream>>>(
                head_part, 2, e->head_b, tab.src, tab.valid, tab.read, raw ? stats : nullptr, tile0, rows, probs, want_logits ? 1 : 0,
                nullptr, 0.0);
            CF_LAUNCHED();
        } else if (n_layers == 0) {
            ProfScope ps(prof, KC_K5_HEAD, stream);
            tc_head_conv_kernel<<<(unsigned)tiles, 256, 0, stream>>>(
                a_in, e->head_w.as<float>(), e->head_b, tab.src, tab.valid, tab.read, raw ? stats : nullptr, tile0, rows, probs, want_logits ? 1 : 0);
            CF_LAUNCHED();
        } else {
            ProfScope ps(prof, KC_K5_HEAD, stream);
            tc_head_kernel<<<(unsigned)tiles, 256, 0, stream>>>(
                head_part, 8, e->head_b, tab.src, tab.valid, tab.read, raw ? stats : nullptr, tile0, rows, probs, want_logits ? 1 : 0,
                bits ? bits->lwords : nullptr, bits ? bits->threshold : 0.0);
            CF_LAUNCHED();
        }
    }
    return CF_OK;
}

__global__ void __launch_bounds__(128, 1)
tc_selftest_f16e5_kernel(const float* __restrict__ a, const uint8_t* __restrict__ wpk, int K, int N, int mode,
                         float* __restrict__ out) {
    extern __shared__ __align__(128) uint8_t smem[];
    uint8_t* a_s = smem;
    uint8_t* w_s = smem + 128 * K * 4;
    uint64_t* bar = reinterpret_cast<uint64_t*>(w_s + (size_t)N * K * 4);
    uint32_t* tmem_slot = reinterpret_cast<uint32_t*>(bar + 1);
    const int row = threadIdx.x, warp = threadIdx.x >> 5;
    if (threadIdx.x == 0) { mbar_init(bar, 1); fence_mbar_init(); }
    if (warp == 0) tmem_alloc<256>(tmem_slot);
    for (int i = threadIdx.x; i < N * K * 4 / 16; i += 128)
        reinterpret_cast<uint4*>(w_s)[i] = reinterpret_cast<const uint4*>(wpk)[i];
    tc_fence_before_sync();
    __syncthreads();
    tc_fence_after_sync();
    const uint32_t tmem = *tmem_slot;
    const uint32_t t_row = tmem + ((uint32_t)(warp * 32) << 16);
    constexpr uint32_t kTmA = 128;
    for (int c = 0; c < K / 16; ++c) {
        float v[16];
        for (int i = 0; i < 16; ++i) v[i] = a[(size_t)row * K + 16 * c + i];
        uint32_t m8[8], lo4[4], hi4[4];
        split_f16e5_chunk(v, m8, lo4, hi4);
        if (mode == 0) {
            *reinterpret_cast<uint4*>(a_s + (2 * c) * 2048 + row * 16) = make_uint4(m8[0], m8[1], m8[2], m8[3]);
            *reinterpret_cast<uint4*>(a_s + (2 * c + 1) * 2048 + row * 16) = make_uint4(m8[4], m8[5], m8[6], m8[7]);
            uint8_t* corr = a_s + 128 * K * 2;
            *reinterpret_cast<uint4*>(corr + (2 * c) * 2048 + row * 16) = make_uint4(lo4[0], lo4[1], lo4[2], lo4[3]);
            *reinterpret_cast<uint4*>(corr + (2 * c + 1) * 2048 + row * 16) = make_uint4(hi4[0], hi4[1], hi4[2], hi4[3]);
        } else {
            uint32_t c8[8] = {lo4[0], lo4[1], lo4[2], lo4[3], hi4[0], hi4[1], hi4[2], hi4[3]};
            tmem_st8_u32(t_row + kTmA + 16 * c, m8);
            tmem_st8_u32(t_row + kTmA + 16 * c + 8, c8);
        }
    }
    fence_proxy_async_smem();
    tmem_st_wait();
    tc_fence_before_sync();
    __syncthreads();
    if (warp == 0) {
        tc_fence_after_sync();
        const uint32_t elected = elect_one();
        const uint32_t a_u = smem_u32(a_s), w_u = smem_u32(w_s);
        const uint32_t id16 = make_idesc_f16(128, N), id8 = make_idesc_e5m2(128, N);
        for (int c = 0; c < K / 16; ++c) {
            const uint64_t bm = make_smem_desc(w_u + c * 2 * (N * 16), N * 16, 128);
            const uint64_t bc = make_smem_desc(w_u + K * N * 2 + c * 2 * (N * 16), N * 16, 128);
            if (mode == 0) {
                umma_bf16_pred(tmem, make_smem_desc(a_u + c * 4096, 2048, 128), bm, id16, c > 0, elected);
                umma_f8_pred(tmem, make_smem_desc(a_u + 128 * K * 2 + c * 4096, 2048, 128), bc, id8, 1, elected);
            } else {
                umma_bf16_ts_pred(tmem, tmem + kTmA + 16 * c, bm, id16, c > 0, elected);
                umma_f8_ts_pred(tmem, tmem + kTmA + 16 * c + 8, bc, id8, 1, elected);
            }
        }
        umma_commit_pred(bar, elected);
    }
    mbar_wait(bar, 0);
    tc_fence_after_sync();
    for (int n0 = 0; n0 < N; n0 += 16) {
        float v[16];
        tmem_ld16(t_row + n0, v);
        for (int i = 0; i < 16; ++i) out[(size_t)row * N + n0 + i] = v[i];
    }
    tc_fence_before_sync();
    __syncthreads();
    if (warp == 0) tmem_dealloc<256>(tmem);
}

int tc_selftest_f16e5(const float* a_dev, int K, int N, const float* w_host, int mode, float* out_dev, cudaStream_t stream) {
    if (K % 16 || K < 16 || K > 64 || N % 16 || N < 16 || N > 128 || (mode != 0 && mode != 1)) {
        set_error("selftest_f16e5: K in {16..64} and N in {16..128}, multiples of 16; mode 0 or 1");
        return CF_ERR_BAD_ARG;
    }
    std::vector<__nv_bfloat16> wpk;
    pack_b_operand_f16e5(w_host, K, N, N, 0, &wpk);
    DevBuf w;
    CF_TRY(w.ensure(wpk.size() * 2));
    CF_CUDA(cudaMemcpyAsync(w.ptr, wpk.data(), wpk.size() * 2, cudaMemcpyHostToDevice, stream));
    const size_t smem = (size_t)128 * K * 4 + (size_t)N * K * 4 + 64;
    CF_CUDA(cudaFuncSetAttribute(tc_selftest_f16e5_kernel, cudaFuncAttributeMaxDynamicSharedMemorySize, (int)smem));
    tc_selftest_f16e5_kernel<<<1, 128, smem, stream>>>(a_dev, w.as<uint8_t>(), K, N, mode, out_dev);
    CF_LAUNCHED();
    CF_CUDA(cudaStreamSynchronize(stream));
    return CF_OK;
}

}
```

### catfish_b200/csrc/tc_ptx.cuh

```cuda
#pragma once

#include <cuda_bf16.h>
#include <cuda_fp16.h>
#include <cuda_fp8.h>
#include <stdint.h>

namespace cf {
namespace ptx {

__device__ __forceinline__ uint32_t smem_u32(const void* p) {
    return static_cast<uint32_t>(__cvta_generic_to_shared(p));
}

__device__ __forceinline__ void mbar_init(uint64_t* bar, uint32_t count) {
    asm volatile("mbarrier.init.shared::cta.b64 [%0], %1;" ::"r"(smem_u32(bar)), "r"(count) : "memory");
}
__device__ __forceinline__ void fence_mbar_init() {
    asm volatile("fence.mbarrier_init.release.cluster;" ::: "memory");
}
__device__ __forceinline__ void mbar_arrive(uint64_t* bar) {
    asm volatile("{\n\t.reg .b64 st;\n\tmbarrier.arrive.shared::cta.b64 st, [%0];\n\t}" ::"r"(smem_u32(bar)) : "memory");
}
__device__ __forceinline__ void mbar_expect_tx(uint64_t* bar, uint32_t bytes) {
    asm volatile("{\n\t.reg .b64 st;\n\tmbarrier.arrive.expect_tx.shared::cta.b64 st, [%0], %1;\n\t}" ::"r"(smem_u32(bar)),
                 "r"(bytes)
                 : "memory");
}
__device__ __forceinline__ bool mbar_try_wait(uint64_t* bar, uint32_t parity) {
    uint32_t ok;
    asm volatile(
        "{\n\t.reg .pred p;\n\t"
        "mbarrier.try_wait.parity.shared::cta.b64 p, [%1], %2;\n\t"
        "selp.u32 %0, 1, 0, p;\n\t}"
        : "=r"(ok)
        : "r"(smem_u32(bar)), "r"(parity)
        : "memory");
    return ok != 0;
}
__device__ __forceinline__ bool mbar_test_wait(uint64_t* bar, uint32_t parity) {
    uint32_t ok;
    asm volatile(
        "{\n\t.reg .pred p;\n\t"
        "mbarrier.test_wait.parity.shared::cta.b64 p, [%1], %2;\n\t"
        "selp.u32 %0, 1, 0, p;\n\t}"
        : "=r"(ok)
        : "r"(smem_u32(bar)), "r"(parity)
        : "memory");
    return ok != 0;
}
__device__ __forceinline__ void mbar_wait(uint64_t* bar, uint32_t parity) {
    while (!mbar_try_wait(bar, parity)) {
    }
}

__device__ __forceinline__ void fence_proxy_async_smem() {
    asm volatile("fence.proxy.async.shared::cta;" ::: "memory");
}
__device__ __forceinline__ void tc_fence_before_sync() {
    asm volatile("tcgen05.fence::before_thread_sync;" ::: "memory");
}
__device__ __forceinline__ void tc_fence_after_sync() {
    asm volatile("tcgen05.fence::after_thread_sync;" ::: "memory");
}

__device__ __forceinline__ void bulk_g2s(void* smem_dst, const void* gmem_src, uint32_t bytes, uint64_t* bar) {
    asm volatile("cp.async.bulk.shared::cluster.global.mbarrier::complete_tx::bytes [%0], [%1], %2, [%3];" ::"r"(
                     smem_u32(smem_dst)),
                 "l"(gmem_src), "r"(bytes), "r"(smem_u32(bar))
                 : "memory");
}

__device__ __forceinline__ void bulk_prefetch_l2(const void* gmem_src, uint32_t bytes) {
    asm volatile("cp.async.bulk.prefetch.L2.global [%0], %1;" ::"l"(gmem_src), "r"(bytes) : "memory");
}

template <int kCols>
__device__ __forceinline__ void tmem_alloc(uint32_t* smem_result) {
    asm volatile("tcgen05.alloc.cta_group::1.sync.aligned.shared::cta.b32 [%0], %1;" ::"r"(smem_u32(smem_result)),
                 "n"(kCols)
                 : "memory");
    asm volatile("tcgen05.relinquish_alloc_permit.cta_group::1.sync.aligned;" ::: "memory");
}
template <int kCols>
__device__ __forceinline__ void tmem_dealloc(uint32_t taddr) {
    asm volatile("tcgen05.dealloc.cta_group::1.sync.aligned.b32 %0, %1;" ::"r"(taddr), "n"(kCols) : "memory");
}

__host__ __device__ constexpr uint64_t make_smem_desc(uint32_t smem_addr, uint32_t lbo_bytes, uint32_t sbo_bytes) {
    uint64_t d = 0;
    d |= (uint64_t)((smem_addr >> 4) & 0x3FFF);
    d |= (uint64_t)((lbo_bytes >> 4) & 0x3FFF) << 16;
    d |= (uint64_t)((sbo_bytes >> 4) & 0x3FFF) << 32;
    d |= (uint64_t)1 << 46;
    return d;
}

__host__ __device__ constexpr uint32_t make_idesc_bf16(int m, int n) {
    return (1u << 4)
           | (1u << 7)
           | (1u << 10)
           | ((uint32_t)(n >> 3) << 17) | ((uint32_t)(m >> 4) << 24);
}

__host__ __device__ constexpr uint32_t make_idesc_f16(int m, int n) {
    return (1u << 4) | ((uint32_t)(n >> 3) << 17) | ((uint32_t)(m >> 4) << 24);
}
__host__ __device__ constexpr uint32_t make_idesc_e5m2(int m, int n) { return make_idesc_bf16(m, n); }

__device__ __forceinline__ void umma_bf16(uint32_t tmem_d, uint64_t adesc, uint64_t bdesc, uint32_t idesc, uint32_t accumulate) {
    asm volatile(
        "{\n\t.reg .pred p;\n\t"
        "setp.ne.b32 p, %4, 0;\n\t"
        "tcgen05.mma.cta_group::1.kind::f16 [%0], %1, %2, %3, p;\n\t}" ::"r"(tmem_d),
        "l"(adesc), "l"(bdesc), "r"(idesc), "r"(accumulate)
        : "memory");
}

__device__ __forceinline__ uint32_t elect_one() {
    uint32_t pred;
    asm volatile("{\n\t.reg .pred p;\n\telect.sync _|p, 0xffffffff;\n\tselp.u32 %0, 1, 0, p;\n\t}" : "=r"(pred));
    return pred;
}
__device__ __forceinline__ void umma_bf16_pred(uint32_t tmem_d, uint64_t adesc, uint64_t bdesc, uint32_t idesc,
                                               uint32_t accumulate, uint32_t elected) {
    asm volatile(
        "{\n\t.reg .pred p, q;\n\t"
        "setp.ne.b32 p, %4, 0;\n\t"
        "setp.ne.b32 q, %5, 0;\n\t"
        "@q tcgen05.mma.cta_group::1.kind::f16 [%0], %1, %2, %3, p;\n\t}" ::"r"(tmem_d),
        "l"(adesc), "l"(bdesc), "r"(idesc), "r"(accumulate), "r"(elected)
        : "memory");
}
__device__ __forceinline__ void umma_bf16_ts_pred(uint32_t tmem_d, uint32_t tmem_a, uint64_t bdesc, uint32_t idesc,
                                                  uint32_t accumulate, uint32_t elected) {
    asm volatile(
        "{\n\t.reg .pred p, q;\n\t"
        "setp.ne.b32 p, %4, 0;\n\t"
        "setp.ne.b32 q, %5, 0;\n\t"
        "@q tcgen05.mma.cta_group::1.kind::f16 [%0], [%1], %2, %3, p;\n\t}" ::"r"(tmem_d),
        "r"(tmem_a), "l"(bdesc), "r"(idesc), "r"(accumulate), "r"(elected)
        : "memory");
}
__device__ __forceinline__ void umma_commit_pred(uint64_t* bar, uint32_t elected) {
    asm volatile(
        "{\n\t.reg .pred q;\n\t"
        "setp.ne.b32 q, %1, 0;\n\t"
        "@q tcgen05.commit.cta_group::1.mbarrier::arrive::one.shared::cluster.b64 [%0];\n\t}" ::"r"(smem_u32(bar)),
        "r"(elected)
        : "memory");
}

__device__ __forceinline__ void umma_f8_pred(uint32_t tmem_d, uint64_t adesc, uint64_t bdesc, uint32_t idesc,
                                             uint32_t accumulate, uint32_t elected) {
    asm volatile(
        "{\n\t.reg .pred p, q;\n\t"
        "setp.ne.b32 p, %4, 0;\n\t"
        "setp.ne.b32 q, %5, 0;\n\t"
        "@q tcgen05.mma.cta_group::1.kind::f8f6f4 [%0], %1, %2, %3, p;\n\t}" ::"r"(tmem_d),
        "l"(adesc), "l"(bdesc), "r"(idesc), "r"(accumulate), "r"(elected)
        : "memory");
}
__device__ __forceinline__ void umma_f8_ts_pred(uint32_t tmem_d, uint32_t tmem_a, uint64_t bdesc, uint32_t idesc,
                                                uint32_t accumulate, uint32_t elected) {
    asm volatile(
        "{\n\t.reg .pred p, q;\n\t"
        "setp.ne.b32 p, %4, 0;\n\t"
        "setp.ne.b32 q, %5, 0;\n\t"
        "@q tcgen05.mma.cta_group::1.kind::f8f6f4 [%0], [%1], %2, %3, p;\n\t}" ::"r"(tmem_d),
        "r"(tmem_a), "l"(bdesc), "r"(idesc), "r"(accumulate), "r"(elected)
        : "memory");
}

__device__ __forceinline__ void umma_bf16_ts(uint32_t tmem_d, uint32_t tmem_a, uint64_t bdesc, uint32_t idesc, uint32_t accumulate) {
    asm volatile(
        "{\n\t.reg .pred p;\n\t"
        "setp.ne.b32 p, %4, 0;\n\t"
        "tcgen05.mma.cta_group::1.kind::f16 [%0], [%1], %2, %3, p;\n\t}" ::"r"(tmem_d),
        "r"(tmem_a), "l"(bdesc), "r"(idesc), "r"(accumulate)
        : "memory");
}

__device__ __forceinline__ void umma_commit(uint64_t* bar) {
    asm volatile("tcgen05.commit.cta_group::1.mbarrier::arrive::one.shared::cluster.b64 [%0];" ::"r"(smem_u32(bar)) : "memory");
}

__device__ __forceinline__ void tmem_ld16(uint32_t taddr, float* v) {
    uint32_t r[16];
    asm volatile(
        "tcgen05.ld.sync.aligned.32x32b.x16.b32 {%0,%1,%2,%3,%4,%5,%6,%7,%8,%9,%10,%11,%12,%13,%14,%15}, [%16];"
        : "=r"(r[0]), "=r"(r[1]), "=r"(r[2]), "=r"(r[3]), "=r"(r[4]), "=r"(r[5]), "=r"(r[6]), "=r"(r[7]), "=r"(r[8]),
          "=r"(r[9]), "=r"(r[10]), "=r"(r[11]), "=r"(r[12]), "=r"(r[13]), "=r"(r[14]), "=r"(r[15])
        : "r"(taddr)
        : "memory");
    asm volatile("tcgen05.wait::ld.sync.aligned;" ::: "memory");
#pragma unroll
    for (int i = 0; i < 16; ++i) v[i] = __uint_as_float(r[i]);
}
__device__ __forceinline__ void tmem_ld16_nowait(uint32_t taddr, uint32_t* r) {
    asm volatile(
        "tcgen05.ld.sync.aligned.32x32b.x16.b32 {%0,%1,%2,%3,%4,%5,%6,%7,%8,%9,%10,%11,%12,%13,%14,%15}, [%16];"
        : "=r"(r[0]), "=r"(r[1]), "=r"(r[2]), "=r"(r[3]), "=r"(r[4]), "=r"(r[5]), "=r"(r[6]), "=r"(r[7]), "=r"(r[8]),
          "=r"(r[9]), "=r"(r[10]), "=r"(r[11]), "=r"(r[12]), "=r"(r[13]), "=r"(r[14]), "=r"(r[15])
        : "r"(taddr)
        : "memory");
}
__device__ __forceinline__ void tmem_ld_wait() { asm volatile("tcgen05.wait::ld.sync.aligned;" ::: "memory"); }
__device__ __forceinline__ void tmem_st16(uint32_t taddr, const float* v) {
    asm volatile(
        "tcgen05.st.sync.aligned.32x32b.x16.b32 [%0], {%1,%2,%3,%4,%5,%6,%7,%8,%9,%10,%11,%12,%13,%14,%15,%16};" ::"r"(taddr),
        "r"(__float_as_uint(v[0])), "r"(__float_as_uint(v[1])), "r"(__float_as_uint(v[2])), "r"(__float_as_uint(v[3])),
        "r"(__float_as_uint(v[4])), "r"(__float_as_uint(v[5])), "r"(__float_as_uint(v[6])), "r"(__float_as_uint(v[7])),
        "r"(__float_as_uint(v[8])), "r"(__float_as_uint(v[9])), "r"(__float_as_uint(v[10])), "r"(__float_as_uint(v[11])),
        "r"(__float_as_uint(v[12])), "r"(__float_as_uint(v[13])), "r"(__float_as_uint(v[14])), "r"(__float_as_uint(v[15]))
        : "memory");
}
__device__ __forceinline__ void tmem_st8_u32(uint32_t taddr, const uint32_t* v) {
    asm volatile("tcgen05.st.sync.aligned.32x32b.x8.b32 [%0], {%1,%2,%3,%4,%5,%6,%7,%8};" ::"r"(taddr), "r"(v[0]), "r"(v[1]),
                 "r"(v[2]), "r"(v[3]), "r"(v[4]), "r"(v[5]), "r"(v[6]), "r"(v[7])
                 : "memory");
}
__device__ __forceinline__ void tmem_st_wait() { asm volatile("tcgen05.wait::st.sync.aligned;" ::: "memory"); }

__device__ __forceinline__ uint64_t pack2(float2 a) {
    uint64_t r;
    asm("mov.b64 %0, {%1, %2};" : "=l"(r) : "f"(a.x), "f"(a.y));
    return r;
}
__device__ __forceinline__ float2 unpack2(uint64_t r) {
    float2 a;
    asm("mov.b64 {%0, %1}, %2;" : "=f"(a.x), "=f"(a.y) : "l"(r));
    return a;
}
__device__ __forceinline__ float2 ffma2(float2 a, float2 b, float2 c) {
    uint64_t d;
    asm("fma.rn.f32x2 %0, %1, %2, %3;" : "=l"(d) : "l"(pack2(a)), "l"(pack2(b)), "l"(pack2(c)));
    return unpack2(d);
}
__device__ __forceinline__ float2 fmul2(float2 a, float2 b) {
    uint64_t d;
    asm("mul.rn.f32x2 %0, %1, %2;" : "=l"(d) : "l"(pack2(a)), "l"(pack2(b)));
    return unpack2(d);
}
__device__ __forceinline__ float2 fadd2(float2 a, float2 b) {
    uint64_t d;
    asm("add.rn.f32x2 %0, %1, %2;" : "=l"(d) : "l"(pack2(a)), "l"(pack2(b)));
    return unpack2(d);
}
__device__ __forceinline__ float2 splat2(float x) { return make_float2(x, x); }

__device__ __forceinline__ void split_bf16(float x, __nv_bfloat16& hi, __nv_bfloat16& lo) {
    hi = __float2bfloat16_rn(x);
    lo = __float2bfloat16_rn(x - __bfloat162float(hi));
}
__device__ __forceinline__ void split_bf16x2(float x0, float x1, uint32_t& hi, uint32_t& lo) {
    const __nv_bfloat162 h = __floats2bfloat162_rn(x0, x1);
    hi = *reinterpret_cast<const uint32_t*>(&h);
    const float2 r = ffma2(make_float2(__uint_as_float(hi << 16), __uint_as_float(hi & 0xffff0000u)), splat2(-1.f),
                           make_float2(x0, x1));
    const __nv_bfloat162 l = __floats2bfloat162_rn(r.x, r.y);
    lo = *reinterpret_cast<const uint32_t*>(&l);
}

constexpr float kCorrScale = 64.f;
__device__ __forceinline__ void split_f16e5x2(float x0, float x1, uint32_t& main, uint32_t& lo) {
    uint32_t h32;
    asm("cvt.rn.satfinite.f16x2.f32 %0, %1, %2;" : "=r"(h32) : "f"(x1), "f"(x0));
    const __half2 m = __hmul2(*reinterpret_cast<const __half2*>(&h32), __floats2half2_rn(1.f / kCorrScale, 1.f / kCorrScale));
    main = *reinterpret_cast<const uint32_t*>(&m);
    const float2 l = ffma2(__half22float2(m), splat2(-kCorrScale * kCorrScale), fmul2(make_float2(x0, x1), splat2(kCorrScale)));
    lo = __nv_cvt_float2_to_fp8x2(l, __NV_SATFINITE, __NV_E5M2);
}
__device__ __forceinline__ uint32_t f16e5_hi4(uint32_t m01, uint32_t m23) { return __byte_perm(m01, m23, 0x7531); }
__device__ __forceinline__ void split_f16e5_chunk(const float* v, uint32_t* main, uint32_t* lo4, uint32_t* hi4) {
#pragma unroll
    for (int j = 0; j < 4; ++j) {
        uint32_t la, lb;
        split_f16e5x2(v[4 * j], v[4 * j + 1], main[2 * j], la);
        split_f16e5x2(v[4 * j + 2], v[4 * j + 3], main[2 * j + 1], lb);
        lo4[j] = la | (lb << 16);
        hi4[j] = f16e5_hi4(main[2 * j], main[2 * j + 1]);
    }
}

__device__ __forceinline__ float ex2_approx(float x) {
    float y;
    asm("ex2.approx.ftz.f32 %0, %1;" : "=f"(y) : "f"(x));
    return y;
}
__device__ __forceinline__ float rcp_approx(float x) {
    float y;
    asm("rcp.approx.ftz.f32 %0, %1;" : "=f"(y) : "f"(x));
    return y;
}
__device__ __forceinline__ float fast_sigmoid(float x) {
    return rcp_approx(1.f + ex2_approx(-1.4426950408889634f * x));
}
__device__ __forceinline__ float fast_tanh(float x) {
    const float e = ex2_approx(-2.8853900817779268f * fabsf(x));
    return copysignf((1.f - e) * rcp_approx(1.f + e), x);
}

__device__ __forceinline__ void rcp4(const float* a, float* inv) {
    const float p01 = a[0] * a[1], p23 = a[2] * a[3];
    const float r = rcp_approx(p01 * p23);
    const float r01 = r * p23, r23 = r * p01;
    inv[0] = r01 * a[1];
    inv[1] = r01 * a[0];
    inv[2] = r23 * a[3];
    inv[3] = r23 * a[2];
}
__device__ __forceinline__ void sigmoid4(const float* x, float* y) {
    float a[4];
#pragma unroll
    for (int i = 0; i < 4; ++i) a[i] = 1.f + ex2_approx(fminf(-1.4426950408889634f * x[i], 28.853900817779268f));
    rcp4(a, y);
}
__device__ __forceinline__ void tanh4(const float* x, float* y) {
    float e[4], a[4], inv[4];
#pragma unroll
    for (int i = 0; i < 4; ++i) {
        e[i] = ex2_approx(-2.8853900817779268f * fabsf(x[i]));
        a[i] = 1.f + e[i];
    }
    rcp4(a, inv);
#pragma unroll
    for (int i = 0; i < 4; ++i) y[i] = copysignf((1.f - e[i]) * inv[i], x[i]);
}

__device__ __forceinline__ float tanh_approx(float x) {
    float y;
    asm("tanh.approx.f32 %0, %1;" : "=f"(y) : "f"(x));
    return y;
}
#ifndef CF_PRECISE_ACT
constexpr float kSigArgScale = -0.34657359027997264f;
constexpr float kTanhArgScale = 0.34657359027997264f;
__device__ __forceinline__ float sigmoid_zb(float acc, float bk) { return fmaf(tanh_approx(fmaf(acc, kSigArgScale, bk)), 0.5f, 0.5f); }
__device__ __forceinline__ float tanh_zb(float acc, float bk) { return tanh_approx(fmaf(acc, kTanhArgScale, bk)); }
__device__ __forceinline__ float2 sigmoid_zb2(float2 acc, float2 bk) {
    const float2 z = ffma2(acc, splat2(kSigArgScale), bk);
    return ffma2(make_float2(tanh_approx(z.x), tanh_approx(z.y)), splat2(0.5f), splat2(0.5f));
}
__device__ __forceinline__ float2 tanh_zb2(float2 acc, float2 bk) {
    const float2 z = ffma2(acc, splat2(kTanhArgScale), bk);
    return make_float2(tanh_approx(z.x), tanh_approx(z.y));
}
#endif
#ifndef CF_PRECISE_ACT
__device__ __forceinline__ void sigmoid4_z(const float* z, float* y) {
#pragma unroll
    for (int i = 0; i < 4; ++i) y[i] = fmaf(tanh_approx(z[i] * -0.34657359027997264f), 0.5f, 0.5f);
}
__device__ __forceinline__ void tanh4_z(const float* z, float* y) {
#pragma unroll
    for (int i = 0; i < 4; ++i) y[i] = tanh_approx(z[i] * 0.34657359027997264f);
}
#else
__device__ __forceinline__ void sigmoid4_z(const float* z, float* y) {
    float a[4];
#pragma unroll
    for (int i = 0; i < 4; ++i) a[i] = 1.f + ex2_approx(fminf(z[i], 28.853900817779268f));
    rcp4(a, y);
}
__device__ __forceinline__ void tanh4_z(const float* z, float* y) {
    float a[4], inv[4];
#pragma unroll
    for (int i = 0; i < 4; ++i) a[i] = 1.f + ex2_approx(fminf(z[i], 28.853900817779268f));
    rcp4(a, inv);
#pragma unroll
    for (int i = 0; i < 4; ++i) y[i] = fmaf(-2.f, inv[i], 1.f);
}
#endif

}
}
```

Baseline: 1.020 billion.

## Fold biases into MMAs via ones-column and rescale GRU weights for tanh activations

```diff
diff --git a/catfish_b200/build.py b/catfish_b200/build.py
--- a/catfish_b200/build.py
+++ b/catfish_b200/build.py
@@ -8,7 +8,7 @@
 INCLUDE = os.path.join(HERE, "..", "include")
 LIB = os.environ.get("CF_LIB_OUT") or os.path.join(HERE, "libcatfish_b200.so")
 SOURCES = ["api.cu", "k1_normalize.cu", "k6_intervals.cu", "k7_chunks.cu", "k8_split.cu", "k9_validate.cu", "k11_sweep.cu", "simt_engine.cu", "tc_engine.cu"]
-NVCC_FLAGS = (["-DCF_PRECISE_ACT"] if os.environ.get("CF_PRECISE_ACT") else []) + os.environ.get("CF_EXTRA_DEFS", "").split() + ["-gencode", "arch=compute_100a,code=sm_100a", "-lineinfo", "-O3", "-std=c++17",
+NVCC_FLAGS = os.environ.get("CF_EXTRA_DEFS", "").split() + ["-gencode", "arch=compute_100a,code=sm_100a", "-lineinfo", "-O3", "-std=c++17",
               "--expt-relaxed-constexpr", "-Xcompiler", "-fPIC,-O2,-Wall", "-Xptxas", "-v"]
 
 
diff --git a/catfish_b200/csrc/tc_engine.cu b/catfish_b200/csrc/tc_engine.cu
--- a/catfish_b200/csrc/tc_engine.cu
+++ b/catfish_b200/csrc/tc_engine.cu
@@ -15,19 +15,25 @@
 constexpr int kC = 32;
 constexpr int kNX = 3 * kH;
 constexpr int kTcChunkTiles = 2368;
-constexpr float kGateScale = -1.4426950408889634f;
-constexpr float kCandScale = 2.8853900817779268f;
+constexpr float kGateArg = 0.5f, kCandArg = 1.f;
+constexpr float kRhScale = 0.5f;
 
 constexpr int kFmtBf16x3 = 0, kFmtF16E5 = 1;
 
 struct ConvParams {
-    static constexpr int kFloats = 10 * 32;
+    static constexpr int kFloats = 4 * 32;
     static constexpr int kW2 = kFloats * 4;
     static constexpr int kW3 = kW2 + 3 * 4096;
     static constexpr int kW45 = kW3 + 4096;
     static constexpr int kW6 = kW45 + 8192;
     static constexpr int kW7 = kW6 + 3 * 4096;
-    static constexpr int kBytes = kW7 + 4096;
+    static constexpr int kB2 = kW7 + 4096;
+    static constexpr int kB3 = kB2 + 1024;
+    static constexpr int kB45 = kB3 + 1024;
+    static constexpr int kB6 = kB45 + 2048;
+    static constexpr int kB7 = kB6 + 1024;
+    static constexpr int kOnes = kB7 + 1024;
+    static constexpr int kBytes = kOnes + 4096;
 };
 
 static void pack_b_operand(const float* w, int K, int N, int ldw, int col0, std::vector<__nv_bfloat16>* out,
@@ -68,11 +74,26 @@
         }
 }
 
+static void put_bias_chunk(__nv_bfloat16* chunk, int col0, const float* b, int n, float scale = 1.f) {
+    for (int j = 0; j < n; ++j) {
+        float r = b[j] * scale;
+        for (int k = 0; k < 3; ++k) {
+            const __nv_bfloat16 p = __float2bfloat16_rn(r);
+            chunk[(size_t)(col0 + j) * 8 + k] = p;
+            r -= __bfloat162float(p);
+        }
+    }
+}
+
+static void put_ones_chunk(__nv_bfloat16* chunk) {
+    for (int m = 0; m < 128; ++m)
+        for (int k = 0; k < 3; ++k) chunk[(size_t)m * 8 + k] = __float2bfloat16_rn(1.f);
+}
+
 struct TcLayer {
     int in = 0;
     DevBuf wfused;
     int fmt = 0;
-    DevBuf bz;
     DevBuf wxz;
 };
 
@@ -172,7 +193,7 @@
             for (float v : g.wgh) wmax = std::max(wmax, std::fabs(v));
             for (float v : g.wch) wmax = std::max(wmax, std::fabs(v));
         }
-        const bool in_range = wmax * kCandScale * kCorrScale < 60000.f;
+        const bool in_range = wmax * std::max(kGateArg, kCandArg) * kCorrScale < 60000.f;
         e->fmt = covered && in_range ? kFmtF16E5 : kFmtBf16x3;
     }
     if (hm.n_res() >= 1) {
@@ -193,8 +214,13 @@
                     lo[idx] = __float2bfloat16_rn(v - __bfloat162float(h));
                 }
         };
+        auto put_b = [&](int off, int col0, const std::vector<float>& b) {
+            put_bias_chunk(reinterpret_cast<__nv_bfloat16*>(blk + off), col0, b.data(), 32);
+        };
         auto put_block1 = [&](int i) {
-            put(6, hm.convs[i].b); put(7, hm.convs[i + 1].b); put(8, hm.convs[i + 2].b); put(9, hm.convs[i + 3].b);
+            put_b(ConvParams::kB45, 0, hm.convs[i].b); put_b(ConvParams::kB45, 32, hm.convs[i + 1].b);
+            put_b(ConvParams::kB6, 0, hm.convs[i + 2].b); put_b(ConvParams::kB7, 0, hm.convs[i + 3].b);
+            put_ones_chunk(reinterpret_cast<__nv_bfloat16*>(blk + ConvParams::kOnes));
             put_w(ConvParams::kW45, hm.convs[i].w.data(), 32, 32, 0, 0, 64);
             put_w(ConvParams::kW45, hm.convs[i + 1].w.data(), 32, 32, 0, 32, 64);
             for (int tap = 0; tap < 3; ++tap) put_w(ConvParams::kW6 + tap * 4096, hm.convs[i + 2].w.data() + tap * 32 * 32, 32, 32, 0, 0, 32);
@@ -202,7 +228,8 @@
         };
         put(0, hm.convs[0].w); put(1, hm.convs[0].b);
         put(2, hm.convs[1].w); put(3, hm.convs[1].b);
-        put(4, hm.convs[2].b); put(5, hm.convs[3].b);
+        put_b(ConvParams::kB2, 0, hm.convs[2].b); put_b(ConvParams::kB3, 0, hm.convs[3].b);
+        put_ones_chunk(reinterpret_cast<__nv_bfloat16*>(blk + ConvParams::kOnes));
         for (int tap = 0; tap < 3; ++tap) put_w(ConvParams::kW2 + tap * 4096, hm.convs[2].w.data() + tap * 32 * 32, 32, 32, 0, 0, 32);
         put_w(ConvParams::kW3, hm.convs[3].w.data(), 32, 32, 0, 0, 32);
         if (hm.n_res() >= 2) put_block1(4);
@@ -223,21 +250,21 @@
         for (int d = 0; d < 2; ++d) {
             const GruDir& g = hm.gru[2 * l + d];
             auto pack = L.fmt == kFmtF16E5 ? pack_b_operand_f16e5 : pack_b_operand;
-            if (L.in > 1) pack(g.wx.data(), L.in, kNX, kNX, 0, &wf, kGateScale, 2 * kH, kCandScale);
-            pack(g.wgh.data(), kH, 2 * kH, 2 * kH, 0, &wf, kGateScale, 1 << 30, 1.f);
-            pack(g.wch.data(), kH, kH, kH, 0, &wf, kCandScale, 1 << 30, 1.f);
+            if (L.in > 1) pack(g.wx.data(), L.in, kNX, kNX, 0, &wf, kGateArg, 2 * kH, kCandArg);
+            pack(g.wgh.data(), kH, 2 * kH, 2 * kH, 0, &wf, kGateArg, 1 << 30, 1.f);
+            pack(g.wch.data(), kH, kH, kH, 0, &wf, kCandArg * kRhScale, 1 << 30, 1.f);
+            const size_t at = wf.size();
+            wf.resize(at + 16 * kNX + 128 * 16, __float2bfloat16_rn(0.f));
+            put_bias_chunk(wf.data() + at, 0, g.bx.data(), 2 * kH, kGateArg);
+            put_bias_chunk(wf.data() + at, 2 * kH, g.bx.data() + 2 * kH, kH, kCandArg);
+            put_ones_chunk(wf.data() + at + 16 * kNX);
         }
         CF_TRY(L.wfused.upload(wf));
-        std::vector<float> bz(2 * kNX);
-        for (int d = 0; d < 2; ++d)
-            for (int j = 0; j < kNX; ++j)
-                bz[d * kNX + j] = hm.gru[2 * l + d].bx[j] * (j < 2 * kH ? kGateScale : kCandScale);
-        CF_TRY(L.bz.upload(bz));
         if (L.in == 1) {
             std::vector<float> wxz(2 * kNX);
             for (int d = 0; d < 2; ++d)
                 for (int j = 0; j < kNX; ++j)
-                    wxz[d * kNX + j] = hm.gru[2 * l + d].wx[j] * (j < 2 * kH ? kGateScale : kCandScale);
+                    wxz[d * kNX + j] = hm.gru[2 * l + d].wx[j] * (j < 2 * kH ? kGateArg : kCandArg);
             CF_TRY(L.wxz.upload(wxz));
         }
     }
@@ -251,7 +278,7 @@
 bool tc_can_emit_bits(const TcEngine* e) { return e && !e->layers.empty(); }
 
 constexpr uint32_t kSliceBytes = 2u * 128 * kC * 2;
-constexpr uint32_t kConvSmem = ConvParams::kBytes + 10 * kSliceBytes + 35 * 128 * 4 + 256;
+constexpr uint32_t kConvSmem = ConvParams::kBytes + 5 * kSliceBytes + 35 * 128 * 4 + 256;
 
 __device__ __forceinline__ void store_a_row16(uint8_t* slice, int row, int c0, const float* v) {
 #pragma unroll
@@ -266,7 +293,13 @@
 }
 
 template <int N>
-__device__ __forceinline__ void conv_mma_pred(uint32_t tmem_d, uint32_t a_slice, uint32_t w_mat, bool first, uint32_t elected) {
+__device__ __forceinline__ void conv_bias_mma(uint32_t tmem_d, uint32_t prm_u, int bias_off, uint32_t elected) {
+    umma_bf16_pred(tmem_d, make_smem_desc(prm_u + ConvParams::kOnes, 2048, 128), make_smem_desc(prm_u + bias_off, N * 16, 128),
+                   make_idesc_bf16(128, N), 0, elected);
+}
+
+template <int N>
+__device__ __forceinline__ void conv_mma_pred(uint32_t tmem_d, uint32_t a_slice, uint32_t w_mat, uint32_t elected) {
     constexpr uint32_t idesc = make_idesc_bf16(128, N);
 #pragma unroll
     for (int pass = 0; pass < 3; ++pass) {
@@ -275,7 +308,7 @@
 #pragma unroll
         for (int kk = 0; kk < 2; ++kk)
             umma_bf16_pred(tmem_d, make_smem_desc(ap + kk * 4096, 2048, 128), make_smem_desc(wp + kk * 2 * (N * 16), N * 16, 128),
-                           idesc, !(first && pass == 0 && kk == 0), elected);
+                           idesc, 1, elected);
     }
 }
 
@@ -287,10 +320,7 @@
     uint8_t* prm = smem;
     uint8_t* o1 = smem + ConvParams::kBytes;
     uint8_t* o2 = o1 + 4 * kSliceBytes;
-    uint8_t* y0 = o2 + kSliceBytes;
-    uint8_t* p1 = y0 + kSliceBytes;
-    uint8_t* p2 = p1 + 3 * kSliceBytes;
-    float* xs = reinterpret_cast<float*>(p2 + kSliceBytes);
+    float* xs = reinterpret_cast<float*>(o2 + kSliceBytes);
     uint64_t* bars = reinterpret_cast<uint64_t*>(xs + 35 * 128);
     uint32_t* tmem_slot = reinterpret_cast<uint32_t*>(bars + 4);
     const float* fp = reinterpret_cast<const float*>(prm);
@@ -326,16 +356,18 @@
                 tc_fence_after_sync();
                 const int t1 = u - 1, t2 = u - 2;
                 if (t1 >= 0 && t1 < kWindow) {
-                    bool first = true;
+                    conv_bias_mma<32>(tmem + 0, prm_u, ConvParams::kB2, elected);
 #pragma unroll
                     for (int tap = 0; tap < 3; ++tap) {
                         const int tt = t1 + tap - 1;
                         if (tt < 0 || tt >= kWindow) continue;
-                        conv_mma_pred<32>(tmem + 0, o1_u + (tt & 3) * kSliceBytes, prm_u + ConvParams::kW2 + tap * 4096, first, elected);
-                        first = false;
-                    }
-                }
-                if (t2 >= 0 && t2 < kWindow) conv_mma_pred<32>(tmem + 32, o2_u, prm_u + ConvParams::kW3, true, elected);
+                        conv_mma_pred<32>(tmem + 0, o1_u + (tt & 3) * kSliceBytes, prm_u + ConvParams::kW2 + tap * 4096, elected);
+                    }
+                }
+                if (t2 >= 0 && t2 < kWindow) {
+                    conv_bias_mma<32>(tmem + 32, prm_u, ConvParams::kB3, elected);
+                    conv_mma_pred<32>(tmem + 32, o2_u, prm_u + ConvParams::kW3, elected);
+                }
                 umma_commit_pred(bar_mma, elected);
             }
         }
@@ -344,15 +376,9 @@
         const int row = q * 32 + lane;
         const int c0 = ch * 16;
         const uint32_t t_lane = tmem + ((uint32_t)(q * 32) << 16) + c0;
-        auto relu_bias = [&](uint32_t* r, int slot, float* v) {
-#pragma unroll
-            for (int i = 0; i < 16; i += 4) {
-                const float4 b4 = *reinterpret_cast<const float4*>(fp + 32 * slot + c0 + i);
-                v[i] = fmaxf(__uint_as_float(r[i]) + b4.x, 0.f);
-                v[i + 1] = fmaxf(__uint_as_float(r[i + 1]) + b4.y, 0.f);
-                v[i + 2] = fmaxf(__uint_as_float(r[i + 2]) + b4.z, 0.f);
-                v[i + 3] = fmaxf(__uint_as_float(r[i + 3]) + b4.w, 0.f);
-            }
+        auto relu = [&](const uint32_t* r, float* v) {
+#pragma unroll
+            for (int i = 0; i < 16; ++i) v[i] = fmaxf(__uint_as_float(r[i]), 0.f);
         };
         auto make_o1 = [&](int t) {
             const float x = xs[t * 128 + row];
@@ -395,9 +421,9 @@
                 tmem_ld_wait();
                 tc_fence_before_sync();
                 float v[16];
-                if (h1) { relu_bias(r1, 4, v); store_a_row16(o2, row, c0, v); }
+                if (h1) { relu(r1, v); store_a_row16(o2, row, c0, v); }
                 if (h2) {
-                    relu_bias(r2, 5, v);
+                    relu(r2, v);
                     const float x = xs[t2 * 128 + row];
 #pragma unroll
                     for (int i = 0; i < 16; ++i) v[i] = fmaxf(v[i] + fmaf(x, fp[c0 + i], fp[32 + c0 + i]), 0.f);
@@ -455,7 +481,7 @@
 constexpr uint32_t kConv4Smem = ConvParams::kBytes + 2 * kSliceBytes + 4 * (32 * 128 * 4) + 35 * 128 * 4 + 256;
 
 template <int N>
-__device__ __forceinline__ void conv_mma_ts_pred(uint32_t tmem_d, uint32_t tmem_a, uint32_t w_mat, bool first, uint32_t elected) {
+__device__ __forceinline__ void conv_mma_ts_pred(uint32_t tmem_d, uint32_t tmem_a, uint32_t w_mat, uint32_t elected) {
     constexpr uint32_t idesc = make_idesc_bf16(128, N);
 #pragma unroll
     for (int pass = 0; pass < 3; ++pass) {
@@ -463,8 +489,7 @@
         const uint32_t wp = w_mat + (pass == 2 ? (uint32_t)(kC * N * 2) : 0u);
 #pragma unroll
         for (int kk = 0; kk < 2; ++kk)
-            umma_bf16_ts_pred(tmem_d, ap + kk * 8, make_smem_desc(wp + kk * 2 * (N * 16), N * 16, 128), idesc,
-                              !(first && pass == 0 && kk == 0), elected);
+            umma_bf16_ts_pred(tmem_d, ap + kk * 8, make_smem_desc(wp + kk * 2 * (N * 16), N * 16, 128), idesc, 1, elected);
     }
 }
 
@@ -523,16 +548,18 @@
                 tc_fence_after_sync();
                 const int t1 = u - 1, t2 = u - 2;
                 if (t1 >= 0 && t1 < kWindow) {
-                    bool first = true;
+                    conv_bias_mma<32>(tmem + 0, prm_u, ConvParams::kB2, elected);
 #pragma unroll
                     for (int tap = 0; tap < 3; ++tap) {
                         const int tt = t1 + tap - 1;
                         if (tt < 0 || tt >= kWindow) continue;
-                        conv_mma_ts_pred<32>(tmem + 0, tmem + kTmO1 + (tt & 3) * 32, prm_u + ConvParams::kW2 + tap * 4096, first, elected);
-                        first = false;
-                    }
-                }
-                if (t2 >= 0 && t2 < kWindow) conv_mma_pred<32>(tmem + 32, o2_u, prm_u + ConvParams::kW3, true, elected);
+                        conv_mma_ts_pred<32>(tmem + 0, tmem + kTmO1 + (tt & 3) * 32, prm_u + ConvParams::kW2 + tap * 4096, elected);
+                    }
+                }
+                if (t2 >= 0 && t2 < kWindow) {
+                    conv_bias_mma<32>(tmem + 32, prm_u, ConvParams::kB3, elected);
+                    conv_mma_pred<32>(tmem + 32, o2_u, prm_u + ConvParams::kW3, elected);
+                }
                 umma_commit_pred(bar_mma_x, elected);
             }
         }
@@ -546,24 +573,27 @@
                 tc_fence_after_sync();
                 const int t3 = u - 3, t4 = u - 5, t5 = u - 6;
                 if (t3 < kWindow) {
+                    conv_bias_mma<64>(tmem + kTmScp1, prm_u, ConvParams::kB45, elected);
                     mbar_wait(&bar_y0_full[ny_slot], ny_par);
                     tc_fence_after_sync();
-                    conv_mma_ts_pred<64>(tmem + kTmScp1, tmem + kTmY0 + ny_slot * 32, prm_u + ConvParams::kW45, true, elected);
+                    conv_mma_ts_pred<64>(tmem + kTmScp1, tmem + kTmY0 + ny_slot * 32, prm_u + ConvParams::kW45, elected);
                     umma_commit_pred(&bar_y0_empty[ny_slot], elected);
                     ++ny;
                     if (++ny_slot == 3) { ny_slot = 0; ny_par ^= 1; }
                 }
                 if (t4 >= 0 && t4 < kWindow) {
-                    bool first = true;
+                    conv_bias_mma<32>(tmem + 64, prm_u, ConvParams::kB6, elected);
 #pragma unroll
                     for (int tap = 0; tap < 3; ++tap) {
                         const int tt = t4 + tap - 1;
                         if (tt < 0 || tt >= kWindow) continue;
-                        conv_mma_ts_pred<32>(tmem + 64, tmem + kTmP1 + (tt % 3) * 32, prm_u + ConvParams::kW6 + tap * 4096, first, elected);
-                        first = false;
-                    }
-                }
-                if (t5 >= 0 && t5 < kWindow) conv_mma_pred<32>(tmem + 96, p2_u, prm_u + ConvParams::kW7, true, elected);
+                        conv_mma_ts_pred<32>(tmem + 64, tmem + kTmP1 + (tt % 3) * 32, prm_u + ConvParams::kW6 + tap * 4096, elected);
+                    }
+                }
+                if (t5 >= 0 && t5 < kWindow) {
+                    conv_bias_mma<32>(tmem + 96, prm_u, ConvParams::kB7, elected);
+                    conv_mma_pred<32>(tmem + 96, p2_u, prm_u + ConvParams::kW7, elected);
+                }
                 umma_commit_pred(bar_mma_y, elected);
             }
         }
@@ -575,17 +605,9 @@
         const uint32_t t_row = tmem + ((uint32_t)(q * 32) << 16);
         const uint32_t t_lane = t_row + c0;
         const uint32_t t_opnd = t_row + ch * 8;
-        auto relu_bias = [&](uint32_t* r, int slot, float* v) {
-#pragma unroll
-            for (int i = 0; i < 16; i += 4) {
-                const float4 b4 = *reinterpret_cast<const float4*>(fp + 32 * slot + c0 + i);
-                const float2 s0 = fadd2(make_float2(__uint_as_float(r[i]), __uint_as_float(r[i + 1])), make_float2(b4.x, b4.y));
-                const float2 s1 = fadd2(make_float2(__uint_as_float(r[i + 2]), __uint_as_float(r[i + 3])), make_float2(b4.z, b4.w));
-                v[i] = fmaxf(s0.x, 0.f);
-                v[i + 1] = fmaxf(s0.y, 0.f);
-                v[i + 2] = fmaxf(s1.x, 0.f);
-                v[i + 3] = fmaxf(s1.y, 0.f);
-            }
+        auto relu = [&](const uint32_t* r, float* v) {
+#pragma unroll
+            for (int i = 0; i < 16; ++i) v[i] = fmaxf(__uint_as_float(r[i]), 0.f);
         };
         if (warp < 8) {
             auto make_o1 = [&](int t) {
@@ -632,7 +654,7 @@
                     if (h2) tmem_ld16_nowait(t_lane + 32, r2);
                     tmem_ld_wait();
                     float v[16];
-                    if (h1) { relu_bias(r1, 4, v); store_a_row16_f<kFmt>(o2, row, c0, v); }
+                    if (h1) { relu(r1, v); store_a_row16_f<kFmt>(o2, row, c0, v); }
                     if (u < kLastX) {
                         fence_proxy_async_smem();
                         tmem_st_wait();
@@ -641,7 +663,7 @@
                         if (lane == 0) mbar_arrive(bar_ready_x);
                     }
                     if (h2) {
-                        relu_bias(r2, 5, v);
+                        relu(r2, v);
                         const float2 x = splat2(xs[t2 * 128 + row]);
 #pragma unroll
                         for (int i = 0; i < 16; i += 2) {
@@ -682,8 +704,8 @@
                     if (h5) tmem_ld16_nowait(t_lane + 96, r5);
                     tmem_ld_wait();
                     float v[16];
-                    if (h3) { relu_bias(r3, 7, v); store_a_tmem16_f<kFmt>(t_opnd + kTmP1 + (t3 % 3) * 32, v); }
-                    if (h4) { relu_bias(r4, 8, v); store_a_row16_f<kFmt>(p2, row, c0, v); }
+                    if (h3) { relu(r3, v); store_a_tmem16_f<kFmt>(t_opnd + kTmP1 + (t3 % 3) * 32, v); }
+                    if (h4) { relu(r4, v); store_a_row16_f<kFmt>(p2, row, c0, v); }
                     fence_proxy_async_smem();
                     tmem_st_wait();
                     tc_fence_before_sync();
@@ -692,10 +714,10 @@
                     if (h3) {
                         float* dst = sc_mine + (t3 & 3) * 4096;
 #pragma unroll
-                        for (int i = 0; i < 16; ++i) dst[i * 128] = __uint_as_float(rs[i]) + fp[192 + c0 + i];
+                        for (int i = 0; i < 16; ++i) dst[i * 128] = __uint_as_float(rs[i]);
                     }
                     if (h5) {
-                        relu_bias(r5, 9, v);
+                        relu(r5, v);
                         const float* sc = sc_mine + (t5 & 3) * 4096;
 #pragma unroll
                         for (int i = 0; i < 16; i += 2) {
@@ -741,7 +763,6 @@
     uint64_t* bar_full = &bars[3];
     uint64_t* bar_empty = &bars[3 + kBlockRing];
     uint32_t* tmem_slot = reinterpret_cast<uint32_t*>(bars + 3 + 2 * kBlockRing);
-    const float* fp = reinterpret_cast<const float*>(prm);
 
     const int warp = threadIdx.x >> 5, lane = threadIdx.x & 31;
     if (threadIdx.x == 0) {
@@ -774,21 +795,24 @@
                 if (u < kWindow) {
                     const uint32_t slot = n % kBlockRing;
                     mbar_wait(&bar_full[slot], (n / kBlockRing) & 1);
-                    conv_mma_pred<64>(tmem + (u & 3) * 64, yin_u + slot * kSliceBytes, prm_u + ConvParams::kW45, true, elected);
+                    conv_bias_mma<64>(tmem + (u & 3) * 64, prm_u, ConvParams::kB45, elected);
+                    conv_mma_pred<64>(tmem + (u & 3) * 64, yin_u + slot * kSliceBytes, prm_u + ConvParams::kW45, elected);
                     umma_commit_pred(&bar_empty[slot], elected);
                     ++n;
                 }
                 if (t2 >= 0 && t2 < kWindow) {
-                    bool first = true;
+                    conv_bias_mma<32>(tmem + kTmP2, prm_u, ConvParams::kB6, elected);
 #pragma unroll
                     for (int tap = 0; tap < 3; ++tap) {
                         const int tt = t2 + tap - 1;
                         if (tt < 0 || tt >= kWindow) continue;
-                        conv_mma_pred<32>(tmem + kTmP2, p1_u + (tt % 3) * kSliceBytes, prm_u + ConvParams::kW6 + tap * 4096, first, elected);
-                        first = false;
-                    }
-                }
-                if (t3 >= 0 && t3 < kWindow) conv_mma_pred<32>(tmem + kTmP3, p2_u, prm_u + ConvParams::kW7, true, elected);
+                        conv_mma_pred<32>(tmem + kTmP2, p1_u + (tt % 3) * kSliceBytes, prm_u + ConvParams::kW6 + tap * 4096, elected);
+                    }
+                }
+                if (t3 >= 0 && t3 < kWindow) {
+                    conv_bias_mma<32>(tmem + kTmP3, prm_u, ConvParams::kB7, elected);
+                    conv_mma_pred<32>(tmem + kTmP3, p2_u, prm_u + ConvParams::kW7, elected);
+                }
                 umma_commit_pred(bar_mma, elected);
             }
         }
@@ -809,17 +833,9 @@
         const int row = q * 32 + lane;
         const int c0 = ch * 16;
         const uint32_t t_lane = tmem + ((uint32_t)(q * 32) << 16) + c0;
-        auto relu_bias = [&](uint32_t* r, int slot, float* v) {
-#pragma unroll
-            for (int i = 0; i < 16; i += 4) {
-                const float4 b4 = *reinterpret_cast<const float4*>(fp + 32 * slot + c0 + i);
-                const float2 s0 = fadd2(make_float2(__uint_as_float(r[i]), __uint_as_float(r[i + 1])), make_float2(b4.x, b4.y));
-                const float2 s1 = fadd2(make_float2(__uint_as_float(r[i + 2]), __uint_as_float(r[i + 3])), make_float2(b4.z, b4.w));
-                v[i] = fmaxf(s0.x, 0.f);
-                v[i + 1] = fmaxf(s0.y, 0.f);
-                v[i + 2] = fmaxf(s1.x, 0.f);
-                v[i + 3] = fmaxf(s1.y, 0.f);
-            }
+        auto relu = [&](const uint32_t* r, float* v) {
+#pragma unroll
+            for (int i = 0; i < 16; ++i) v[i] = fmaxf(__uint_as_float(r[i]), 0.f);
         };
         uint32_t it = 0;
         if (lane == 0) mbar_arrive(bar_ready);
@@ -838,19 +854,17 @@
                 }
                 tmem_ld_wait();
                 float v[16];
-                if (h1) { relu_bias(r1, 7, v); store_a_row16_f<kFmt>(p1 + (u % 3) * kSliceBytes, row, c0, v); }
-                if (h2) { relu_bias(r2, 8, v); store_a_row16_f<kFmt>(p2, row, c0, v); }
+                if (h1) { relu(r1, v); store_a_row16_f<kFmt>(p1 + (u % 3) * kSliceBytes, row, c0, v); }
+                if (h2) { relu(r2, v); store_a_row16_f<kFmt>(p2, row, c0, v); }
                 fence_proxy_async_smem();
                 tc_fence_before_sync();
                 __syncwarp();
                 if (lane == 0) mbar_arrive(bar_ready);
                 if (h3) {
-                    relu_bias(r3, 9, v);
+                    relu(r3, v);
 #pragma unroll
                     for (int i = 0; i < 16; i += 2) {
-                        const float2 sc = fadd2(make_float2(__uint_as_float(rs[i]), __uint_as_float(rs[i + 1])),
-                                                *reinterpret_cast<const float2*>(fp + 192 + c0 + i));
-                        const float2 o = fadd2(make_float2(v[i], v[i + 1]), sc);
+                        const float2 o = fadd2(make_float2(v[i], v[i + 1]), make_float2(__uint_as_float(rs[i]), __uint_as_float(rs[i + 1])));
                         v[i] = fmaxf(o.x, 0.f);
                         v[i + 1] = fmaxf(o.y, 0.f);
                     }
@@ -871,10 +885,12 @@
     static constexpr uint32_t kWx = 0;
     static constexpr uint32_t kWgh = kWx + (kNoX ? 0u : 2u * KX * kNX * 2);
     static constexpr uint32_t kWch = kWgh + 2u * kH * 128 * 2;
-    static constexpr uint32_t kWBytes = kWch + 2u * kH * 64 * 2;
+    static constexpr uint32_t kBiasChunk = kWch + 2u * kH * 64 * 2;
+    static constexpr uint32_t kOnes = kBiasChunk + 16u * kNX * 2;
+    static constexpr uint32_t kWBytes = kOnes + 128u * 16 * 2;
     static constexpr uint32_t kRing = kWBytes;
-    static constexpr uint32_t kBias = kRing + (uint32_t)kStages * 8192;
-    static constexpr uint32_t kBars = kBias + 2 * 192 * 4;
+    static constexpr uint32_t kXw = kRing + (uint32_t)kStages * 8192;
+    static constexpr uint32_t kBars = kXw + 192 * 4;
     static constexpr uint32_t kSmem = kBars + 512;
     static constexpr int kBarG = 0, kBarC = 1, kBarRh = 2, kBarH = 3, kBarCfree = 4, kBarXdone = 5;
     static constexpr int kBarFull = 16, kBarEmpty = 16 + kStages, kBarTma = 16 + 2 * kStages, kBarW = 16 + 3 * kStages;
@@ -886,8 +902,7 @@
 
 template <int KX, int FMT, int FMT_OUT>
 __global__ void __launch_bounds__(kGruF2Threads, 1)
-tc_gru_fused2_kernel(const uint8_t* __restrict__ wpk, const float* __restrict__ bias,
-                     const __nv_bfloat16* __restrict__ x_blocks, __nv_bfloat16* __restrict__ y_out,
+tc_gru_fused2_kernel(const uint8_t* __restrict__ wpk, const __nv_bfloat16* __restrict__ x_blocks, __nv_bfloat16* __restrict__ y_out,
                      const float* __restrict__ head_w, float* __restrict__ head_part, int n_tiles,
                      long long* __restrict__ trace, const float* __restrict__ x_scalar, const float* __restrict__ wx_scalar) {
     using Cfg = GruF2Cfg<KX>;
@@ -914,7 +929,7 @@
     uint64_t* bars = reinterpret_cast<uint64_t*>(smem + Cfg::kBars);
     uint64_t* w_bar = &bars[Cfg::kBarW];
     uint32_t* tmem_slot = reinterpret_cast<uint32_t*>(&bars[Cfg::kBarW + 1]);
-    float* bias_s = reinterpret_cast<float*>(smem + Cfg::kBias);
+    float* xw_s = reinterpret_cast<float*>(smem + Cfg::kXw);
 
     const int warp = threadIdx.x >> 5, lane = threadIdx.x & 31;
     const int dir = blockIdx.x & 1;
@@ -947,13 +962,7 @@
         mbar_init(w_bar, 1);
         fence_mbar_init();
     }
-#ifndef CF_PRECISE_ACT
-    if (threadIdx.x < 192) bias_s[threadIdx.x] = bias[dir * kNX + threadIdx.x] * (threadIdx.x < 2 * kH ? kSigArgScale : kTanhArgScale);
-    if (kNoX && threadIdx.x < 192) bias_s[192 + threadIdx.x] = wx_scalar[dir * kNX + threadIdx.x] * (threadIdx.x < 2 * kH ? kSigArgScale : kTanhArgScale);
-#else
-    if (threadIdx.x < 192) bias_s[threadIdx.x] = bias[dir * kNX + threadIdx.x];
-    if (kNoX && threadIdx.x < 192) bias_s[192 + threadIdx.x] = wx_scalar[dir * kNX + threadIdx.x];
-#endif
+    if (kNoX && threadIdx.x < kNX) xw_s[threadIdx.x] = wx_scalar[dir * kNX + threadIdx.x];
     if (warp == 16) tmem_alloc<512>(tmem_slot);
     tc_fence_before_sync();
     __syncthreads();
@@ -1040,6 +1049,7 @@
             constexpr uint32_t idesc_x = kE5 ? make_idesc_f16(128, kNX) : make_idesc_bf16(128, kNX);
             constexpr uint32_t idesc_g8 = make_idesc_e5m2(128, 2 * kH), idesc_c8 = make_idesc_e5m2(128, kH);
             constexpr uint32_t idesc_x8 = make_idesc_e5m2(128, kNX);
+            constexpr uint32_t idesc_bias = make_idesc_bf16(128, kNX);
             const uint32_t elected = elect_one();
             const int c = warp - 16;
             const uint32_t s0 = smem_u32(smem);
@@ -1056,6 +1066,15 @@
                 else if (gs > 0 && gs - 1 < total1) mbar_wait(&bars[8 + Cfg::kBarXdone], (gs - 1) & 1);
                 if (gs > 0) mbar_wait(&b[Cfg::kBarCfree], (gs - 1) & 1);
                 if (lane == 0) CF_TR(c, gs, 10);
+                {
+                    uint32_t ones_lo = (uint32_t)make_smem_desc(s0 + Cfg::kOnes, 2048, 128);
+                    uint32_t bias_lo = (uint32_t)make_smem_desc(s0 + Cfg::kBiasChunk, kNX * 16, 128);
+                    asm volatile("" : "+r"(ones_lo), "+r"(bias_lo));
+                    constexpr uint64_t ahi = make_smem_desc(0, 2048, 128) & 0xffffffff00000000ull;
+                    constexpr uint64_t bhi = make_smem_desc(0, kNX * 16, 128) & 0xffffffff00000000ull;
+                    tc_fence_after_sync();
+                    umma_bf16_pred(dg, ahi | ones_lo, bhi | bias_lo, idesc_bias, 0, elected);
+                }
                 auto issue_x = [&](auto st0c) {
                     constexpr int kSt0 = decltype(st0c)::value;
                     static_assert(kSt0 + Cfg::kChunks <= Cfg::kStages || kNoX, "an entry does not wrap around the ring");
@@ -1073,13 +1092,13 @@
                         tc_fence_after_sync();
                         const uint32_t a_lo = ring_lo + st * (8192 >> 4), w_lo = wx_lo + kk * (2 * kNX * 16 >> 4);
                         if (kE5) {
-                            umma_bf16_pred(dg, ahi | a_lo, bhi | w_lo, idesc_x, kk != 0, elected);
+                            umma_bf16_pred(dg, ahi | a_lo, bhi | w_lo, idesc_x, 1, elected);
                             umma_f8_pred(dg, ahi | (a_lo + (4096 >> 4)), bhi | (w_lo + (KX * kNX * 2 >> 4)), idesc_x8, 1, elected);
                         } else {
 #pragma unroll
                             for (int pass = 0; pass < 3; ++pass)
                                 umma_bf16_pred(dg, ahi | (a_lo + (pass == 1 ? 4096 >> 4 : 0)),
-                                               bhi | (w_lo + (pass == 2 ? KX * kNX * 2 >> 4 : 0)), idesc_x, (kk | pass) != 0, elected);
+                                               bhi | (w_lo + (pass == 2 ? KX * kNX * 2 >> 4 : 0)), idesc_x, 1, elected);
                         }
                         umma_commit_pred(&bars[Cfg::kBarEmpty + st], elected);
                         if (lane == 0) CF_TRC(c, gs, 20 + kk);
@@ -1112,7 +1131,7 @@
 #pragma unroll
                     for (int kk = 0; kk < kH / 16; ++kk) {
                         const uint32_t w_lo = wgh_lo + kk * (2 * 128 * 16 >> 4);
-                        umma_bf16_ts_pred(dg, ta + kk * 8, ghi | w_lo, idesc_g, !kNoX || kk != 0, elected);
+                        umma_bf16_ts_pred(dg, ta + kk * 8, ghi | w_lo, idesc_g, 1, elected);
                         umma_f8_ts_pred(dg, ta + 32 + kk * 8, ghi | (w_lo + (kH * 128 * 2 >> 4)), idesc_g8, 1, elected);
                     }
                 } else {
@@ -1122,7 +1141,7 @@
 #pragma unroll
                         for (int kk = 0; kk < kH / 16; ++kk)
                             umma_bf16_ts_pred(dg, ap + kk * 8, ghi | (wgh_lo + (pass == 2 ? kH * 128 * 2 >> 4 : 0) + kk * (2 * 128 * 16 >> 4)),
-                                              idesc_g, !kNoX || (pass | kk) != 0, elected);
+                                              idesc_g, 1, elected);
                     }
                 }
                 umma_commit_pred(&b[Cfg::kBarG], elected);
@@ -1134,7 +1153,7 @@
 #pragma unroll
                     for (int kk = 0; kk < kH / 16; ++kk) {
                         const uint32_t w_lo = wch_lo + kk * (2 * 64 * 16 >> 4);
-                        umma_bf16_ts_pred(dc, ta + kk * 8, chi | w_lo, idesc_c, !kNoX || kk != 0, elected);
+                        umma_bf16_ts_pred(dc, ta + kk * 8, chi | w_lo, idesc_c, 1, elected);
                         umma_f8_ts_pred(dc, ta + 32 + kk * 8, chi | (w_lo + (kH * 64 * 2 >> 4)), idesc_c8, 1, elected);
                     }
                 } else {
@@ -1144,7 +1163,7 @@
 #pragma unroll
                         for (int kk = 0; kk < kH / 16; ++kk)
                             umma_bf16_ts_pred(dc, ap + kk * 8, chi | (wch_lo + (pass == 2 ? kH * 64 * 2 >> 4 : 0) + kk * (2 * 64 * 16 >> 4)),
-                                              idesc_c, !kNoX || (pass | kk) != 0, elected);
+                                              idesc_c, 1, elected);
                     }
                 }
                 umma_commit_pred(&b[Cfg::kBarC], elected);
@@ -1176,37 +1195,26 @@
 #pragma unroll
             for (int j = 0; j < 8; ++j) h2[c][j] = make_float2(0.f, 0.f);
 
-        auto bias4 = [&](int idx, float xv) -> float4 {
-            float4 b4 = *reinterpret_cast<const float4*>(bias_s + idx);
+        auto arg4 = [&](const uint32_t* a, int idx, float xv, float2& z0, float2& z1) {
+            z0 = make_float2(__uint_as_float(a[0]), __uint_as_float(a[1]));
+            z1 = make_float2(__uint_as_float(a[2]), __uint_as_float(a[3]));
             if (kNoX) {
-                const float4 w4 = *reinterpret_cast<const float4*>(bias_s + 192 + idx);
-                b4.x = fmaf(xv, w4.x, b4.x); b4.y = fmaf(xv, w4.y, b4.y); b4.z = fmaf(xv, w4.z, b4.z); b4.w = fmaf(xv, w4.w, b4.w);
-            }
-            return b4;
+                const float4 w4 = *reinterpret_cast<const float4*>(xw_s + idx);
+                z0 = ffma2(splat2(xv), make_float2(w4.x, w4.y), z0);
+                z1 = ffma2(splat2(xv), make_float2(w4.z, w4.w), z1);
+            }
         };
-        auto sig4 = [&](const uint32_t* a, float4 b4, float2& o0, float2& o1) {
-#ifndef CF_PRECISE_ACT
-            o0 = sigmoid_zb2(make_float2(__uint_as_float(a[0]), __uint_as_float(a[1])), make_float2(b4.x, b4.y));
-            o1 = sigmoid_zb2(make_float2(__uint_as_float(a[2]), __uint_as_float(a[3])), make_float2(b4.z, b4.w));
-#else
-            float z[4] = {__uint_as_float(a[0]) + b4.x, __uint_as_float(a[1]) + b4.y, __uint_as_float(a[2]) + b4.z, __uint_as_float(a[3]) + b4.w};
-            float y[4];
-            sigmoid4_z(z, y);
-            o0 = make_float2(y[0], y[1]);
-            o1 = make_float2(y[2], y[3]);
-#endif
+        auto sig4 = [&](const uint32_t* a, int idx, float xv, float2& o0, float2& o1) {
+            float2 z0, z1;
+            arg4(a, idx, xv, z0, z1);
+            o0 = ffma2(make_float2(tanh_approx(z0.x), tanh_approx(z0.y)), splat2(0.5f), splat2(0.5f));
+            o1 = ffma2(make_float2(tanh_approx(z1.x), tanh_approx(z1.y)), splat2(0.5f), splat2(0.5f));
         };
-        auto tanh4v = [&](const uint32_t* a, float4 b4, float2& o0, float2& o1) {
-#ifndef CF_PRECISE_ACT
-            o0 = tanh_zb2(make_float2(__uint_as_float(a[0]), __uint_as_float(a[1])), make_float2(b4.x, b4.y));
-            o1 = tanh_zb2(make_float2(__uint_as_float(a[2]), __uint_as_float(a[3])), make_float2(b4.z, b4.w));
-#else
-            float z[4] = {__uint_as_float(a[0]) + b4.x, __uint_as_float(a[1]) + b4.y, __uint_as_float(a[2]) + b4.z, __uint_as_float(a[3]) + b4.w};
-            float y[4];
-            tanh4_z(z, y);
-            o0 = make_float2(y[0], y[1]);
-            o1 = make_float2(y[2], y[3]);
-#endif
+        auto tanh4v = [&](const uint32_t* a, int idx, float xv, float2& o0, float2& o1) {
+            float2 z0, z1;
+            arg4(a, idx, xv, z0, z1);
+            o0 = make_float2(tanh_approx(z0.x), tanh_approx(z0.y));
+            o1 = make_float2(tanh_approx(z1.x), tanh_approx(z1.y));
         };
         auto begin_tile = [&](int c) {
             const uint32_t t_ahi = t_row + c * 256 + 3 * kH + j0 / 2, t_alo = t_ahi + 32;
@@ -1235,9 +1243,9 @@
             uint32_t hi[8], lo[8];
 #pragma unroll
             for (int i = 0; i < 16; i += 4) {
-                float2 r0, r1;
-                sig4(ar + i, bias4(j0 + i, xv), r0, r1);
-                const float2 p0 = fmul2(r0, h2[c][i >> 1]), p1 = fmul2(r1, h2[c][(i >> 1) + 1]);
+                float2 t0, t1;
+                tanh4v(ar + i, j0 + i, xv, t0, t1);
+                const float2 p0 = ffma2(t0, h2[c][i >> 1], h2[c][i >> 1]), p1 = ffma2(t1, h2[c][(i >> 1) + 1], h2[c][(i >> 1) + 1]);
                 split4<FMT>(p0.x, p0.y, p1.x, p1.y, i, hi, lo);
             }
             tmem_st8_u32(t_ahi, hi);
@@ -1261,7 +1269,7 @@
                 tmem_ld16_nowait(t_acc + kH, au);
                 tmem_ld_wait();
 #pragma unroll
-                for (int i = 0; i < 16; i += 4) sig4(au + i, bias4(kH + j0 + i, xv), u2[i >> 1], u2[(i >> 1) + 1]);
+                for (int i = 0; i < 16; i += 4) sig4(au + i, kH + j0 + i, xv, u2[i >> 1], u2[(i >> 1) + 1]);
             }
             if (warp == 0 && lane == 0) CF_TR(2 + c, gs, 52);
             mbar_wait(&b[Cfg::kBarC], gs & 1);
@@ -1277,7 +1285,7 @@
 #pragma unroll
             for (int i = 0; i < 16; i += 4) {
                 float2 c0v, c1v;
-                tanh4v(ac + i, bias4(2 * kH + j0 + i, xv), c0v, c1v);
+                tanh4v(ac + i, 2 * kH + j0 + i, xv, c0v, c1v);
                 float2& ha = h2[c][i >> 1];
                 float2& hb = h2[c][(i >> 1) + 1];
                 ha = ffma2(u2[i >> 1], ffma2(c0v, splat2(-1.f), ha), c0v);
@@ -1540,23 +1548,23 @@
             if (L.in == 1) {
                 if (L.fmt == kFmtF16E5)
                     tc_gru_fused2_kernel<1, 1, 1><<<grid2, kGruF2Threads, GruF2Cfg<1>::kSmem, stream>>>(
-                        L.wfused.as<uint8_t>(), L.bz.as<float>(), nullptr, yo, hw_l, hp_l, (int)tiles, nullptr, feat, L.wxz.as<float>());
+                        L.wfused.as<uint8_t>(), nullptr, yo, hw_l, hp_l, (int)tiles, nullptr, feat, L.wxz.as<float>());
                 else
                     tc_gru_fused2_kernel<1, 0, 0><<<grid2, kGruF2Threads, GruF2Cfg<1>::kSmem, stream>>>(
-                        L.wfused.as<uint8_t>(), L.bz.as<float>(), nullptr, yo, hw_l, hp_l, (int)tiles, nullptr, feat, L.wxz.as<float>());
+                        L.wfused.as<uint8_t>(), nullptr, yo, hw_l, hp_l, (int)tiles, nullptr, feat, L.wxz.as<float>());
             } else if (L.in == kC) {
                 if (fmt_out == kFmtF16E5)
                     tc_gru_fused2_kernel<32, 0, 1><<<grid2, kGruF2Threads, GruF2Cfg<32>::kSmem, stream>>>(
-                        L.wfused.as<uint8_t>(), L.bz.as<float>(), a_in, yo, hw_l, hp_l, (int)tiles, nullptr, nullptr, nullptr);
+                        L.wfused.as<uint8_t>(), a_in, yo, hw_l, hp_l, (int)tiles, nullptr, nullptr, nullptr);
                 else
                     tc_gru_fused2_kernel<32, 0, 0><<<grid2, kGruF2Threads, GruF2Cfg<32>::kSmem, stream>>>(
-                        L.wfused.as<uint8_t>(), L.bz.as<float>(), a_in, yo, hw_l, hp_l, (int)tiles, nullptr, nullptr, nullptr);
+                        L.wfused.as<uint8_t>(), a_in, yo, hw_l, hp_l, (int)tiles, nullptr, nullptr, nullptr);
             } else if (L.fmt == kFmtF16E5) {
                 tc_gru_fused2_kernel<128, 1, 1><<<grid2, kGruF2Threads, GruF2Cfg<128>::kSmem, stream>>>(
-                    L.wfused.as<uint8_t>(), L.bz.as<float>(), a_in, yo, hw_l, hp_l, (int)tiles, trace_dev, nullptr, nullptr);
+                    L.wfused.as<uint8_t>(), a_in, yo, hw_l, hp_l, (int)tiles, trace_dev, nullptr, nullptr);
             } else {
                 tc_gru_fused2_kernel<128, 0, 0><<<grid2, kGruF2Threads, GruF2Cfg<128>::kSmem, stream>>>(
-                    L.wfused.as<uint8_t>(), L.bz.as<float>(), a_in, yo, hw_l, hp_l, (int)tiles, trace_dev, nullptr, nullptr);
+                    L.wfused.as<uint8_t>(), a_in, yo, hw_l, hp_l, (int)tiles, trace_dev, nullptr, nullptr);
             }
             CF_LAUNCHED();
 #ifdef CF_TRACE_PROBES
diff --git a/catfish_b200/csrc/tc_ptx.cuh b/catfish_b200/csrc/tc_ptx.cuh
--- a/catfish_b200/csrc/tc_ptx.cuh
+++ b/catfish_b200/csrc/tc_ptx.cuh
@@ -282,95 +282,11 @@
     }
 }
 
-__device__ __forceinline__ float ex2_approx(float x) {
-    float y;
-    asm("ex2.approx.ftz.f32 %0, %1;" : "=f"(y) : "f"(x));
-    return y;
-}
-__device__ __forceinline__ float rcp_approx(float x) {
-    float y;
-    asm("rcp.approx.ftz.f32 %0, %1;" : "=f"(y) : "f"(x));
-    return y;
-}
-__device__ __forceinline__ float fast_sigmoid(float x) {
-    return rcp_approx(1.f + ex2_approx(-1.4426950408889634f * x));
-}
-__device__ __forceinline__ float fast_tanh(float x) {
-    const float e = ex2_approx(-2.8853900817779268f * fabsf(x));
-    return copysignf((1.f - e) * rcp_approx(1.f + e), x);
-}
-
-__device__ __forceinline__ void rcp4(const float* a, float* inv) {
-    const float p01 = a[0] * a[1], p23 = a[2] * a[3];
-    const float r = rcp_approx(p01 * p23);
-    const float r01 = r * p23, r23 = r * p01;
-    inv[0] = r01 * a[1];
-    inv[1] = r01 * a[0];
-    inv[2] = r23 * a[3];
-    inv[3] = r23 * a[2];
-}
-__device__ __forceinline__ void sigmoid4(const float* x, float* y) {
-    float a[4];
-#pragma unroll
-    for (int i = 0; i < 4; ++i) a[i] = 1.f + ex2_approx(fminf(-1.4426950408889634f * x[i], 28.853900817779268f));
-    rcp4(a, y);
-}
-__device__ __forceinline__ void tanh4(const float* x, float* y) {
-    float e[4], a[4], inv[4];
-#pragma unroll
-    for (int i = 0; i < 4; ++i) {
-        e[i] = ex2_approx(-2.8853900817779268f * fabsf(x[i]));
-        a[i] = 1.f + e[i];
-    }
-    rcp4(a, inv);
-#pragma unroll
-    for (int i = 0; i < 4; ++i) y[i] = copysignf((1.f - e[i]) * inv[i], x[i]);
-}
-
 __device__ __forceinline__ float tanh_approx(float x) {
     float y;
     asm("tanh.approx.f32 %0, %1;" : "=f"(y) : "f"(x));
     return y;
 }
-#ifndef CF_PRECISE_ACT
-constexpr float kSigArgScale = -0.34657359027997264f;
-constexpr float kTanhArgScale = 0.34657359027997264f;
-__device__ __forceinline__ float sigmoid_zb(float acc, float bk) { return fmaf(tanh_approx(fmaf(acc, kSigArgScale, bk)), 0.5f, 0.5f); }
-__device__ __forceinline__ float tanh_zb(float acc, float bk) { return tanh_approx(fmaf(acc, kTanhArgScale, bk)); }
-__device__ __forceinline__ float2 sigmoid_zb2(float2 acc, float2 bk) {
-    const float2 z = ffma2(acc, splat2(kSigArgScale), bk);
-    return ffma2(make_float2(tanh_approx(z.x), tanh_approx(z.y)), splat2(0.5f), splat2(0.5f));
-}
-__device__ __forceinline__ float2 tanh_zb2(float2 acc, float2 bk) {
-    const float2 z = ffma2(acc, splat2(kTanhArgScale), bk);
-    return make_float2(tanh_approx(z.x), tanh_approx(z.y));
-}
-#endif
-#ifndef CF_PRECISE_ACT
-__device__ __forceinline__ void sigmoid4_z(const float* z, float* y) {
-#pragma unroll
-    for (int i = 0; i < 4; ++i) y[i] = fmaf(tanh_approx(z[i] * -0.34657359027997264f), 0.5f, 0.5f);
-}
-__device__ __forceinline__ void tanh4_z(const float* z, float* y) {
-#pragma unroll
-    for (int i = 0; i < 4; ++i) y[i] = tanh_approx(z[i] * 0.34657359027997264f);
-}
-#else
-__device__ __forceinline__ void sigmoid4_z(const float* z, float* y) {
-    float a[4];
-#pragma unroll
-    for (int i = 0; i < 4; ++i) a[i] = 1.f + ex2_approx(fminf(z[i], 28.853900817779268f));
-    rcp4(a, y);
-}
-__device__ __forceinline__ void tanh4_z(const float* z, float* y) {
-    float a[4], inv[4];
-#pragma unroll
-    for (int i = 0; i < 4; ++i) a[i] = 1.f + ex2_approx(fminf(z[i], 28.853900817779268f));
-    rcp4(a, inv);
-#pragma unroll
-    for (int i = 0; i < 4; ++i) y[i] = fmaf(-2.f, inv[i], 1.f);
-}
-#endif
-
-}
-}
+
+}
+}
```

Result: faster. 1.059 billion, median of 6 (+3.8%).
